# ajpowelsnl/mhm2_proxy

Measured on AMD Instinct MI355X. Metric: k-mers/s (whole node), k=21 150bp reads, higher is better.
Workload: dtype u64

## Files before the change

mhm2_proxy_amd/csrc/kcount_kernels.hip:

```cpp
#include <hip/hip_runtime.h>
#include <type_traits>

#include <algorithm>

#include "kcount_launch.hpp"
#include "kmer_ops.hpp"

namespace mhm {

template <int NL>
constexpr int kTile() {
  return TILE_BASES[NL];
}
template <int NL>
constexpr int kEThreads() {
  return E_THREADS_NL[NL];
}
template <int NL>
constexpr int kPTile() {
  return P_TILE[NL];
}
template <int NL>
constexpr int kPThreads() {
  return P_THREADS[NL];
// ... 1210 lines not shown
#pragma unroll
  for (int j = 0; j < W; j++) {
    const uint32_t i = threadIdx.x + j * NT;
    const uint64_t idx = ch.start + (i < ch.count ? i : ch.count - 1);
    if (RecKind<NL, CMP>::C32) {
      rk[j][0] = (uint64_t)gload((const uint32_t *)src.w[0] + idx);
      rx[j] = (uint32_t)gload(src.ext + idx);
      continue;
    }
    if (RecKind<NL, CMP>::M2) {
      const u32x4 v = gload4((const uint32_t *)src.w[0] + 4 * idx);
      rk[j][0] = (uint64_t)v.x | ((uint64_t)v.y << 32);
      rk[j][NL - 1] = (uint64_t)v.z | ((uint64_t)v.w << 32);
      rx[j] = 0u;
      continue;
    }
#pragma unroll
    for (int w = 0; w < NL; w++) rk[j][w] = gload(src.w[w] + idx);
    rx[j] = PACKED ? 0u : (uint32_t)gload(src.ext + idx);
  }
  if (RecKind<NL, CMP>::C32) {
#pragma unroll
    for (int j = 0; j < W; j++) rk[j][0] |= (uint64_t)rx[j] << 32;
  }
#pragma unroll
  for (int j = 0; j < W; j++) re[j] = PACKED ? (uint32_t)(rk[j][RecKind<NL, CMP>::XW] & 63u) : rx[j];
}

template <int NL, bool PACKED, bool CMP>
__global__ __launch_bounds__(kPThreads<NL>()) void k_part_hist(PartitionParams p) {
  constexpr int NT = kPThreads<NL>(), T = kPTile<NL>(), W = T / NT;
  extern __shared__ __align__(16) uint32_t hist[];
  const uint32_t nf = 1u << p.fine_bits;
  for (uint32_t b = threadIdx.x; b < nf; b += NT) hist[b] = 0;
  uint32_t c;
  if (!xcd_chunk(p, c)) return;
  const SChunk ch = chunk_of<T>(p, c);
  const PlaneSet src = p.srcs[ch.src];
  uint64_t rk[W][NL];
  uint32_t re[W];
  load_chunk<NL, PACKED, CMP, W>(src, ch, rk, re);
  __syncthreads();
#pragma unroll
  for (int j = 0; j < W; j++) {
    if (threadIdx.x + j * NT < ch.count) atomicAdd(&hist[fine_digit<NL, PACKED, CMP>(rk[j], p)], 1u);
  }
  __syncthreads();
  unsigned long long *g = p.fine_hist + (uint64_t)ch.coarse_local * nf;
  for (uint32_t b = threadIdx.x; b < nf; b += NT) {
    const uint32_t c = hist[b];
    if (c) atomicAdd(&g[b], (unsigned long long)c);
  }
}

template <int NL, bool PACKED, bool CMP, int BPT = 8>
__global__ __launch_bounds__(kPThreads<NL>()) void k_part_scatter(PartitionParams p) {
  constexpr int NT = kPThreads<NL>(), T = kPTile<NL>(), W = T / NT;
  static_assert(T % NT == 0 && NT % 64 == 0, "whole records per thread, whole waves");
  extern __shared__ __align__(16) unsigned char smem[];
  const uint32_t nf = 1u << p.fine_bits;
  scatter_clear<NT>((uint32_t *)smem, nf);
  uint32_t c;
  if (!xcd_chunk(p, c)) return;
  const SChunk ch = chunk_of<T>(p, c);
  const PlaneSet src = p.srcs[ch.src];
  if constexpr (RecKind<NL, CMP>::C32) {
    const uint32_t *b32 = (const uint32_t *)src.w[0] + ch.start;
    const uint8_t *b8 = src.ext + ch.start;
    uint32_t lo[W], hi[W];
#pragma unroll
    for (int j = 0; j < W; j++) {
      const uint32_t i = min((uint32_t)(threadIdx.x + j * NT), ch.count - 1u);
      lo[j] = gload(b32 + i);
      hi[j] = gload(b8 + i);
    }
    const uint64_t cmask = (1ull << (EXT_BITS + 2 * p.k - p.coarse_bits - p.fine_bits)) - 1;
#pragma unroll
    for (int j = 0; j < W; j++) {
      uint64_t r[1] = {(uint64_t)lo[j] | ((uint64_t)hi[j] << 32)};
      hi[j] = (threadIdx.x + j * NT < ch.count) ? (1u << 31) | fine_digit<NL, PACKED, CMP>(r, p) : 0u;
      lo[j] = (uint32_t)(r[0] & cmask);
    }
    BinLimit lim{0, 0, 0};
    if (p.coarse_fcap) {
      const uint64_t fc = p.coarse_fcap[ch.coarse_local];
      lim = BinLimit{p.coarse_base[ch.coarse_local], fc, fc};
    }
    __syncthreads();
    scatter_staged_c40<W, NT, false, BPT>(lo, hi, nf, smem, smem + staged_cnt_bytes(nf),
                                     p.fine_cursor + (uint64_t)ch.coarse_local * nf, p.out, lim, p.err);
    return;
  }
  uint64_t rk[W][NL];
  uint32_t re[W], inf[W];
  load_chunk<NL, PACKED, CMP, W>(src, ch, rk, re);
  const uint64_t cmask =
      (1ull << (EXT_BITS + (NL == 1 ? 2 * p.k : RecKind<NL, CMP>::lw(p.k)) - p.coarse_bits - p.fine_bits)) - 1;
#pragma unroll
  for (int j = 0; j < W; j++) {
    inf[j] = (threadIdx.x + j * NT < ch.count)
                 ? ((1u << 31) | (re[j] << 16) | fine_digit<NL, PACKED, CMP>(rk[j], p))
                 : 0u;
    if (CMP) rk[j][0] &= cmask;
  }
  __syncthreads();
  BinLimit lim{0, 0, 0};
  if (p.coarse_fcap) {
    const uint64_t fc = p.coarse_fcap[ch.coarse_local];
    lim = BinLimit{p.coarse_base[ch.coarse_local], fc, fc};
  }
  unsigned long long *cur = p.fine_cursor + (uint64_t)ch.coarse_local * nf;
  constexpr int SF = RecKind<NL, CMP>::M2 ? SF_AOS2 : SF_WORDS;
  scatter_staged<NL, PACKED, W, SF, NT, W * NT, BPT>(rk, inf, nf, smem, smem + staged_cnt_bytes(nf), cur, 1, p.out, lim, p.err);
}

template <int NL, bool PACKED, bool CMP>
__global__ __launch_bounds__(kPThreads<NL>()) void k_sketch(PartitionParams p, unsigned int *hll, unsigned int *fhist) {
  constexpr int NT = kPThreads<NL>(), T = kPTile<NL>(), W = T / NT;
  __shared__ unsigned int reg[SKETCH_M];
  __shared__ unsigned int fh[SKETCH_FH];
  __shared__ unsigned int s_ext;
  if (threadIdx.x == 0) s_ext = 0;
  for (int i = threadIdx.x; i < SKETCH_M; i += NT) reg[i] = 0;
  if (fhist)
    for (int i = threadIdx.x; i < SKETCH_FH; i += NT) fh[i] = 0;
  const SChunk ch = chunk_of<T>(p, blockIdx.x);
  const PlaneSet src = p.srcs[ch.src];
  uint64_t rk[W][NL];
  uint32_t re[W];
  load_chunk<NL, PACKED, CMP, W>(src, ch, rk, re);
  __syncthreads();
  const uint64_t low_mask = CMP ? 63ull : PACKED ? (1ull << (EXT_BITS + p.hbits)) - 1 : 0ull;
  uint32_t ext_adds = 0;
#pragma unroll
  for (int j = 0; j < W; j++) {
    if (threadIdx.x + j * NT >= ch.count) continue;
    ext_adds += (uint32_t)(((re[j] >> 3) & 7u) < 4u) + (uint32_t)((re[j] & 7u) < 4u);
    uint64_t h = 0x9E3779B97F4A7C15ull;
#pragma unroll
    for (int w = 0; w < NL; w++) h = fmix64(h ^ (w == RecKind<NL, CMP>::XW ? rk[j][w] & ~low_mask : rk[j][w]));
    const uint32_t rho = (uint32_t)__clzll(h | (uint64_t)(SKETCH_M - 1)) + 1;
    atomicMax(&reg[h & (SKETCH_M - 1)], rho);
    if (fhist) atomicAdd(&fh[fine_digit<NL, PACKED, CMP>(rk[j], p)], 1u);
  }
  atomicAdd(&s_ext, ext_adds);
  __syncthreads();
  if (fhist)
    for (int i = threadIdx.x; i < SKETCH_FH; i += NT)
      if (fh[i]) atomicAdd(&fhist[i], fh[i]);
  for (int i = threadIdx.x; i < SKETCH_M; i += NT)
    if (reg[i]) {
      atomicMax(&hll[i], reg[i]);
      if (!(blockIdx.x & 1u)) atomicMax(&hll[SKETCH_M + 1 + i], reg[i]);
    }
  if (threadIdx.x == 0 && s_ext) atomicAdd(&hll[SKETCH_M], s_ext);
}

__global__ void k_init_fine(const unsigned long long *coarse_base, const unsigned long long *coarse_fcap, uint32_t n_coarse,
                            int fine_bits, unsigned long long *base, unsigned long long *cursor) {
  const uint64_t i = (uint64_t)blockIdx.x * blockDim.x + threadIdx.x;
  if (i >= ((uint64_t)n_coarse << fine_bits)) return;
  const uint64_t c = i >> fine_bits, d = i & ((1ull << fine_bits) - 1);
  const unsigned long long b = coarse_base[c] + d * coarse_fcap[c];
  base[i] = b;
  cursor[i] = b;
}

__global__ __launch_bounds__(256) void k_count_windows(ReadsView rv, int k, unsigned long long *out, unsigned int *err) {
  __shared__ unsigned long long s_acc[4];
  unsigned long long acc = 0;
  bool bad = false;
  const uint64_t stride = (uint64_t)gridDim.x * blockDim.x;
  for (uint64_t r0 = (uint64_t)blockIdx.x * blockDim.x + threadIdx.x; r0 < rv.n_reads; r0 += 4 * stride) {
    uint64_t a[4], b[4];
#pragma unroll
    for (int u = 0; u < 4; u++) {
      const uint64_t r = r0 + u * stride, rr = r < rv.n_reads ? r : rv.n_reads - 1;
      a[u] = rv.offs[rr];
      b[u] = rv.offs[rr + 1];
    }
#pragma unroll
    for (int u = 0; u < 4; u++) {
      if (r0 + u * stride >= rv.n_reads) break;
      bad |= b[u] < a[u] || b[u] - a[u] > 65535;
      const uint64_t L = b[u] - a[u];
      acc += (b[u] >= a[u] && L > (uint64_t)k + 1) ? L - k - 1 : 0;
    }
  }
  if (blockIdx.x == 0 && threadIdx.x == 0)
    bad |= rv.offs[0] != rv.obase + rv.head || rv.offs[rv.n_reads] - rv.obase != rv.n_bases;
  if (bad) atomicOr(err, 4u);
  acc = wave_sum_u64(acc);
  if ((threadIdx.x & 63) == 0) s_acc[threadIdx.x >> 6] = acc;
  __syncthreads();
  if (threadIdx.x == 0) {
    const unsigned long long t = s_acc[0] + s_acc[1] + s_acc[2] + s_acc[3];
    if (t) atomicAdd(out, t);
  }
}

__global__ __launch_bounds__(256) void k_expand_nibbles(const uint8_t *nib, uint8_t *arena, uint64_t b0, uint64_t n) {
  const uint64_t a0 = b0 & ~15ull, end = b0 + n;
  const uint64_t p0 = a0 + ((uint64_t)blockIdx.x * blockDim.x + threadIdx.x) * 16;
  if (p0 >= end) return;
  uint32_t w[4] = {0, 0, 0, 0};
#pragma unroll
  for (int i = 0; i < 16; i++) {
    const uint64_t p = p0 + i;
    if (p >= b0 && p < end) {
      const uint64_t j = p - b0;
      const uint32_t v = (nib[j >> 1] >> (4 * (uint32_t)(j & 1))) & 15u;
      w[i >> 2] |= ((v & 7u) | ((v >> 3) * 0xf8u)) << (8 * (i & 3));
    }
  }
  if (p0 >= b0 && p0 + 16 <= end) {
    *(uint4 *)(arena + p0) = make_uint4(w[0], w[1], w[2], w[3]);
    return;
  }
#pragma unroll
  for (int i = 0; i < 16; i++) {
    const uint64_t p = p0 + i;
    if (p >= b0 && p < end) arena[p] = (uint8_t)(w[i >> 2] >> (8 * (i & 3)));
  }
}

__global__ __launch_bounds__(256) void k_offs_from_deltas(const uint32_t *d, uint64_t *offs, uint64_t n, uint64_t b0) {
  for (uint64_t i = (uint64_t)blockIdx.x * 256 + threadIdx.x; i < n; i += (uint64_t)gridDim.x * 256) offs[i] = b0 + d[i];
}

__global__ __launch_bounds__(1024) void k_scan(const unsigned long long *in, unsigned long long *base,
                                               unsigned long long *cursor, uint32_t n) {
  __shared__ unsigned long long wsum[17];
  const int tid = threadIdx.x, lane = tid & 63, wid = tid >> 6;
  const uint32_t per = (n + 1023) / 1024;
  const uint32_t lo = min((uint32_t)tid * per, n), hi = min(lo + per, n);
  unsigned long long s = 0;
  for (uint32_t i = lo; i < hi; i++) s += (in[i] + 3) & ~3ull;
  unsigned long long x = s;
#pragma unroll
  for (int d = 1; d < 64; d <<= 1) {
    unsigned long long y = __shfl_up(x, d, 64);
    if (lane >= d) x += y;
  }
  if (lane == 63) wsum[wid] = x;
  __syncthreads();
  if (tid == 0) {
    unsigned long long acc = 0;
    for (int w = 0; w < 16; w++) {
      unsigned long long t = wsum[w];
      wsum[w] = acc;
      acc += t;
    }
  }
  __syncthreads();
  unsigned long long run = wsum[wid] + x - s;
  for (uint32_t i = lo; i < hi; i++) {
    base[i] = run;
    cursor[i] = run;
    run += (in[i] + 3) & ~3ull;
  }
}


template <int NL>
constexpr int count_rpt() {
  return NL == 1 ? 4 : 1;
}

template <int NL>
__device__ __forceinline__ uint32_t slot_hash(const uint64_t *key) {
  if (NL == 1) {
    const uint32_t x = (uint32_t)(key[0] >> 32) * 0x9E3779B1u + (uint32_t)key[0] * 0x85EBCA77u;
    return x ^ (x >> 15);
  }
  uint64_t h = key[0] * 0x9E3779B97F4A7C15ull;
#pragma unroll
  for (int w = 1; w < NL; w++) h = (h ^ (h >> 31) ^ key[w]) * 0xC2B2AE3D27D4EB4Full;
  h ^= h >> 29;
  return (uint32_t)(h >> 32);
}

__device__ __forceinline__ int cmp_group(uint32_t key, int kshl, uint32_t ng) {
  return (int)(__umul24((key << kshl) >> 16, ng) >> 16);
}

template <typename K>
struct CountLds {
  K *keys;
  uint32_t *cnt;
  uint32_t *ext;
  int cap;
  uint32_t *clog;
};

typedef __attribute__((address_space(3))) unsigned int lds_u32_t;
__device__ __forceinline__ uint32_t lds_add_late(unsigned int *p, uint32_t v) {
  lds_u32_t *q = (lds_u32_t *)p;
  asm volatile("" : "+v"(q));
  return __hip_atomic_fetch_add(q, v, __ATOMIC_RELAXED, __HIP_MEMORY_SCOPE_WORKGROUP);
}

#ifndef MHMKC_TAIL_DIV
#define MHMKC_TAIL_DIV 1
#endif
#ifndef MHMKC_TAIL_SLOTS
#define MHMKC_TAIL_SLOTS 4
// ... 1115 lines not shown
  const size_t lds = ((size_t)1 << p.fine_bits) * 4;
  hipError_t e = allow_lds(k_part_hist<NL, PK, CMP>, lds);
  if (e != hipSuccess) return e;
  k_part_hist<NL, PK, CMP><<<dim3(p.grid), dim3(kPThreads<NL>()), lds, s>>>(p);
  return hipGetLastError();
}

template <int NL, bool PK, bool CMP = false>
static hipError_t do_part_scatter(const PartitionParams &p, hipStream_t s) {
  const uint32_t nf = 1u << p.fine_bits;
  const size_t lds = staged_cnt_bytes(nf) + staged_area_bytes(NL, kPTile<NL>(), PK, RecKind<NL, CMP>::C32 ? SF_C32 : SF_WORDS);
  if (nf <= (uint32_t)kPThreads<NL>()) {
    hipError_t e = allow_lds(k_part_scatter<NL, PK, CMP, 1>, lds);
    if (e != hipSuccess) return e;
    k_part_scatter<NL, PK, CMP, 1><<<dim3(p.grid), dim3(kPThreads<NL>()), lds, s>>>(p);
    return hipGetLastError();
  }
  hipError_t e = allow_lds(k_part_scatter<NL, PK, CMP>, lds);
  if (e != hipSuccess) return e;
  k_part_scatter<NL, PK, CMP><<<dim3(p.grid), dim3(kPThreads<NL>()), lds, s>>>(p);
  return hipGetLastError();
}

template <int NL, bool PK, bool CMP = false>
static hipError_t do_count(const CountParams &p, hipStream_t s) {
  const size_t lds = count_lds_bytes(NL, RecKind<NL, CMP>::C32);
  const uint32_t grid = p.grid && p.grid < p.n_buckets ? p.grid : p.n_buckets;
  hipError_t e = p.wide_thr ? allow_lds(k_count<NL, PK, CMP, true>, lds) : allow_lds(k_count<NL, PK, CMP, false>, lds);
  if (e != hipSuccess) return e;
  if (p.wide_thr)
    k_count<NL, PK, CMP, true><<<dim3(grid), dim3(C_THREADS), lds, s>>>(p);
  else
    k_count<NL, PK, CMP, false><<<dim3(grid), dim3(C_THREADS), lds, s>>>(p);
  return hipGetLastError();
}

hipError_t launch_tile_first_read(const ReadsView &r, uint32_t *out, uint32_t n_tiles, int tile, hipStream_t s) {
  if (!n_tiles) return hipSuccess;
  k_tile_first_read<<<dim3((n_tiles + 255) / 256), dim3(256), 0, s>>>(r, out, n_tiles, tile);
  return hipGetLastError();
}

uint64_t read_start_words(uint64_t n_tiles, int nl) {
  const uint64_t T = nl == 1 ? kTile<1>() : nl == 2 ? kTile<2>() : nl == 3 ? kTile<3>() : kTile<4>();
  const uint64_t NG = nl == 1 ? kGroups<1>() : nl == 2 ? kGroups<2>() : nl == 3 ? kGroups<3>() : kGroups<4>();
  return n_tiles * (T / 32) + NG + 2;
}

hipError_t launch_read_start_bits(const ReadsView &r, uint32_t *bits, uint64_t n_words, hipStream_t s) {
  const uint64_t blocks = std::min<uint64_t>(8192, (r.n_reads + 1 + 255) / 256);
  k_read_start_bits<<<dim3((unsigned)blocks), dim3(256), 0, s>>>(r, bits, n_words);
  return hipGetLastError();
}

hipError_t launch_count_windows(const ReadsView &r, int k, unsigned long long *out, unsigned int *err, hipStream_t s) {
  if (!r.n_reads) return hipSuccess;
  const uint64_t blocks = std::min<uint64_t>(2048, (r.n_reads + 1023) / 1024);
  k_count_windows<<<dim3((unsigned)blocks), dim3(256), 0, s>>>(r, k, out, err);
  return hipGetLastError();
}

hipError_t launch_offs_from_deltas(const uint32_t *d, uint64_t *offs, uint64_t n, uint64_t b0, hipStream_t s) {
  if (!n) return hipSuccess;
  k_offs_from_deltas<<<dim3((unsigned)std::min<uint64_t>(4096, (n + 255) / 256)), dim3(256), 0, s>>>(d, offs, n, b0);
  return hipGetLastError();
}

hipError_t launch_expand_nibbles(const uint8_t *nib, uint8_t *arena, uint64_t b0, uint64_t n, hipStream_t s) {
  if (!n) return hipSuccess;
  const uint64_t blocks16 = (b0 + n - (b0 & ~15ull) + 15) / 16;
  k_expand_nibbles<<<dim3((unsigned)((blocks16 + 255) / 256)), dim3(256), 0, s>>>(nib, arena, b0, n);
  return hipGetLastError();
}

__global__ __launch_bounds__(256) void k_inc_fixup(const unsigned long long *coarse_base,
                                                  const unsigned long long *coarse_fcap, int fine_bits,
                                                  unsigned long long *cursor, uint8_t *skip, unsigned int *err) {
  const uint32_t c = blockIdx.x, nf = 1u << fine_bits;
  const unsigned long long b0 = coarse_base[c], fcap = coarse_fcap[c];
  unsigned long long *cur = cursor + ((uint64_t)c << fine_bits);
  int over = 0;
  for (uint32_t f = threadIdx.x; f < nf; f += 256) over |= cur[f] > b0 + (f + 1) * fcap;
  over = __syncthreads_or(over);
  if (over)
    for (uint32_t f = threadIdx.x; f < nf; f += 256) cur[f] = b0 + f * fcap;
  if (threadIdx.x == 0) {
    skip[c] = (uint8_t)over;
    if (c == 0) atomicAnd(err, ~2u);
  }
}

hipError_t launch_inc_fixup(const unsigned long long *coarse_base, const unsigned long long *coarse_fcap,
                            uint32_t n_coarse, int fine_bits, unsigned long long *cursor, uint8_t *skip,
                            unsigned int *err, hipStream_t s) {
  if (!n_coarse) return hipSuccess;
  k_inc_fixup<<<dim3(n_coarse), dim3(256), 0, s>>>(coarse_base, coarse_fcap, fine_bits, cursor, skip, err);
  return hipGetLastError();
}

hipError_t launch_init_fine(const unsigned long long *coarse_base, const unsigned long long *coarse_fcap,
                            uint32_t n_coarse, int fine_bits, unsigned long long *base, unsigned long long *cursor,
                            hipStream_t s) {
  const uint64_t n = (uint64_t)n_coarse << fine_bits;
  if (!n) return hipSuccess;
  k_init_fine<<<dim3((unsigned)((n + 255) / 256)), dim3(256), 0, s>>>(coarse_base, coarse_fcap, n_coarse, fine_bits,
                                                                      base, cursor);
  return hipGetLastError();
}

hipError_t launch_extract_hist(const ExtractParams &p, int nl, bool packed, hipStream_t s) {
  if (!p.n_tiles) return hipSuccess;
  if (p.compact) return MHM_DISPATCH_MIXED(nl, do_extract_hist, (p, s));
  MHM_DISPATCH(nl, packed, do_extract_hist, (p, s));
}

hipError_t launch_extract_scatter(const ExtractParams &p, int nl, bool packed, hipStream_t s) {
  if (!p.n_tiles) return hipSuccess;
  if (p.compact) return MHM_DISPATCH_MIXED(nl, do_extract_scatter, (p, s));
  MHM_DISPATCH(nl, packed, do_extract_scatter, (p, s));
}

hipError_t launch_part_hist(const PartitionParams &p, int nl, bool packed, hipStream_t s) {
  if (!p.n_chunks) return hipSuccess;
  if (p.compact) return MHM_DISPATCH_MIXED(nl, do_part_hist, (p, s));
  MHM_DISPATCH(nl, packed, do_part_hist, (p, s));
}

hipError_t launch_part_scatter(const PartitionParams &p, int nl, bool packed, hipStream_t s) {
  if (!p.n_chunks) return hipSuccess;
  if (p.compact) return MHM_DISPATCH_MIXED(nl, do_part_scatter, (p, s));
  MHM_DISPATCH(nl, packed, do_part_scatter, (p, s));
}

hipError_t launch_chunk_runs(const SRun *runs, uint32_t n_runs, SChunk *chunks, int tile, hipStream_t s) {
  if (!n_runs) return hipSuccess;
  k_chunk_runs<<<dim3(n_runs), dim3(256), 0, s>>>(runs, chunks, tile);
  return hipGetLastError();
}

template <int NL, bool PK, bool CMP = false>
static hipError_t do_sketch(const PartitionParams &p, uint32_t n, unsigned int *hll, bool fh, hipStream_t s) {
  k_sketch<NL, PK, CMP><<<dim3(n), dim3(kPThreads<NL>()), 0, s>>>(p, hll, fh ? hll + SKETCH_WORDS : nullptr);
  return hipGetLastError();
}

hipError_t launch_sketch(const PartitionParams &p, uint32_t n_chunks, unsigned int *hll, int nl, bool packed,
                         hipStream_t s, bool fine_hist) {
  if (!n_chunks) return hipSuccess;
  if (fine_hist && p.fine_bits != SKETCH_FB) return hipErrorInvalidValue;
  if (p.compact) return MHM_DISPATCH_MIXED(nl, do_sketch, (p, n_chunks, hll, fine_hist, s));
  MHM_DISPATCH(nl, packed, do_sketch, (p, n_chunks, hll, fine_hist, s));
}

hipError_t launch_scan(const unsigned long long *in, unsigned long long *base, unsigned long long *cursor, uint32_t n,
                       hipStream_t s) {
  k_scan<<<dim3(1), dim3(1024), 0, s>>>(in, base, cursor, n);
  return hipGetLastError();
}

hipError_t launch_count(const CountParams &p, int nl, bool packed, hipStream_t s) {
  if (!p.n_buckets) return hipSuccess;
  if (p.compact) return MHM_DISPATCH_MIXED(nl, do_count, (p, s));
  MHM_DISPATCH(nl, packed, do_count, (p, s));
}


template <typename V>
__global__ __launch_bounds__(256) void k_seg_gather(const SegCopy *segs, const V *src, V *dst) {
  const SegCopy sc = segs[blockIdx.x];
  const V *s = src + sc.src;
  V *d = dst + sc.dst;
  for (uint64_t i = threadIdx.x; i < sc.n; i += 256) d[i] = s[i];
}

hipError_t launch_seg_gather(const SegCopy *segs, uint32_t n_segs, const void *src, void *dst, int elem_bytes,
                             hipStream_t s) {
  if (!n_segs) return hipSuccess;
  const dim3 grid(n_segs), block(256);
  switch (elem_bytes) {
    case 1: k_seg_gather<uint8_t><<<grid, block, 0, s>>>(segs, (const uint8_t *)src, (uint8_t *)dst); break;
    case 4: k_seg_gather<uint32_t><<<grid, block, 0, s>>>(segs, (const uint32_t *)src, (uint32_t *)dst); break;
    case 8: k_seg_gather<uint2><<<grid, block, 0, s>>>(segs, (const uint2 *)src, (uint2 *)dst); break;
    case 16: k_seg_gather<uint4><<<grid, block, 0, s>>>(segs, (const uint4 *)src, (uint4 *)dst); break;
    default: return hipErrorInvalidValue;
  }
  return hipGetLastError();
}


template <int NL>
static hipError_t do_smer_owner(const SmerParams &p, hipStream_t s) {
  const size_t lds = smer_owner_lds<NL>(p.n_ranks);
  hipError_t e = allow_lds(k_smer_owner<NL>, lds);
  if (e != hipSuccess) return e;
  k_smer_owner<NL><<<dim3(p.n_tiles), dim3(kEThreads<NL>()), lds, s>>>(p);
  return hipGetLastError();
}

template <int NL>
static hipError_t do_smer_pack(const SmerParams &p, hipStream_t s) {
  const size_t lds = smer_pack_lds<NL>(p.n_ranks);
  hipError_t e = allow_lds(k_smer_pack<NL>, lds);
  if (e != hipSuccess) return e;
  k_smer_pack<NL><<<dim3(p.n_tiles), dim3(kEThreads<NL>()), lds, s>>>(p);
  return hipGetLastError();
}

hipError_t launch_smer_owner(const SmerParams &p, int nl, hipStream_t s) {
  if (!p.n_tiles) return hipSuccess;
  if (p.n_ranks < 2 || p.n_ranks > 255 || p.m < 1 || p.m > 28 || p.m > p.k) return hipErrorInvalidValue;
  switch (nl) {
    case 2: return do_smer_owner<2>(p, s);
    case 3: return do_smer_owner<3>(p, s);
    case 4: return do_smer_owner<4>(p, s);
  }
  return hipErrorInvalidValue;
}

hipError_t launch_smer_pack(const SmerParams &p, int nl, hipStream_t s) {
  if (!p.n_tiles) return hipSuccess;
  if (p.n_ranks < 2 || p.n_ranks > 255) return hipErrorInvalidValue;
  switch (nl) {
    case 2: return do_smer_pack<2>(p, s);
    case 3: return do_smer_pack<3>(p, s);
    case 4: return do_smer_pack<4>(p, s);
  }
  return hipErrorInvalidValue;
}

template <int NL, bool PK, bool CMP, bool HIST>
static hipError_t do_smer_extract(const ExtractParams &p, const SmerSource &src, hipStream_t s) {
  constexpr int T = kTile<NL>();
  constexpr int SF = RecKind<NL, CMP>::M2 ? SF_AOS2 : SF_WORDS;
  const size_t lds = HIST ? (size_t)p.n_bins * 4 : staged_cnt_bytes(p.n_bins) + staged_area_bytes(NL, T, PK, SF);
  hipError_t e = allow_lds(k_smer_extract<NL, PK, CMP, HIST>, lds);
  if (e != hipSuccess) return e;
  k_smer_extract<NL, PK, CMP, HIST><<<dim3(p.n_tiles), dim3(kEThreads<NL>()), lds, s>>>(p, src);
  return hipGetLastError();
}

template <bool HIST>
static hipError_t smer_extract_nl(const ExtractParams &p, const SmerSource &src, int nl, bool packed, hipStream_t s) {
  if (p.compact)
    return nl == 2 ? do_smer_extract<2, true, true, HIST>(p, src, s) : nl == 3 ? do_smer_extract<3, true, true, HIST>(p, src, s)
         : nl == 4 ? do_smer_extract<4, true, true, HIST>(p, src, s) : hipErrorInvalidValue;
  switch (nl * 2 + (packed ? 1 : 0)) {
    case 4: return do_smer_extract<2, false, false, HIST>(p, src, s);
    case 5: return do_smer_extract<2, true, false, HIST>(p, src, s);
    case 6: return do_smer_extract<3, false, false, HIST>(p, src, s);
    case 7: return do_smer_extract<3, true, false, HIST>(p, src, s);
    case 8: return do_smer_extract<4, false, false, HIST>(p, src, s);
    case 9: return do_smer_extract<4, true, false, HIST>(p, src, s);
  }
  return hipErrorInvalidValue;
}

hipError_t launch_smer_extract(const ExtractParams &p, const SmerSource &src, int nl, bool packed, bool hist,
                               hipStream_t s) {
  if (!p.n_tiles) return hipSuccess;
  return hist ? smer_extract_nl<true>(p, src, nl, packed, s) : smer_extract_nl<false>(p, src, nl, packed, s);
}

hipError_t launch_smer_rebase(uint64_t *desc, uint64_t n, uint64_t delta, unsigned long long *nwin, hipStream_t s) {
  if (!n) return hipSuccess;
  k_smer_rebase<<<dim3((unsigned)std::min<uint64_t>(4096, (n + 255) / 256)), dim3(256), 0, s>>>(desc, n, delta, nwin);
  return hipGetLastError();
}

hipError_t launch_smer_tiles(const uint64_t *wpre, uint64_t n_smer, uint64_t *tile_first, uint32_t n_tiles, int tile,
                             hipStream_t s) {
  if (!n_smer) return hipSuccess;
  k_smer_tiles<<<dim3((n_tiles + 1 + 255) / 256), dim3(256), 0, s>>>(wpre, n_smer, tile_first, n_tiles, tile);
  return hipGetLastError();
}

}
```

mhm2_proxy_amd/csrc/kcount_launch.hpp:

```cpp
#pragma once
#include <hip/hip_runtime.h>
#include <stdint.h>

namespace mhm {

struct ReadsView {
  const uint8_t *bytes;
  const uint64_t *offs;
  uint64_t n_reads;
  uint64_t n_bases;
  uint64_t obase;
  uint32_t head;
  uint32_t pad;
};

struct PlaneSet {
  uint64_t *w[4];
  uint8_t *ext;
};

struct ExtractParams {
  ReadsView reads;
  const uint32_t *tile_first_read;
  uint32_t n_tiles;
// ... 67 lines not shown
  uint32_t xcd_start[9];
  uint32_t grid;
  const PlaneSet *srcs;
  int k;
  int coarse_bits;
  int fine_bits;
  int hbits;
  int compact;
  unsigned long long *fine_hist;
  unsigned long long *fine_cursor;
  const unsigned long long *coarse_base;
  const unsigned long long *coarse_fcap;
  unsigned int *err;
  PlaneSet out;
};

struct CountParams {
  PlaneSet recs;
  const unsigned long long *bucket_base;
  const unsigned long long *bucket_end;
  int hbits;
  int compact;
  int coarse_bits, fine_bits;
  uint32_t bucket0;
  uint32_t n_buckets;
  uint32_t grid;
  int k;
  int cap;
  int dmin_thres;
  double dyn_mult;
  int wide_thr;
  int nlo;
  uint64_t *out_keys;
  uint16_t *out_counts;
  char *out_left;
  char *out_right;
  unsigned long long *out_cursor;
  unsigned long long out_cap;
  unsigned long long *stats;
  unsigned int *err;
  uint64_t ctg_n;
  const uint64_t *ctg_keys[4];
  const uint32_t *ctg_state;
  const uint32_t *ctg_bucket;
  uint32_t ctg_base;
  PlaneSet spill;
  uint8_t *ctg_done;
  const uint8_t *coarse_skip;
};

__host__ __device__ inline uint32_t ctg_state_word(uint32_t count, uint32_t l, uint32_t r) {
  return (count & 0xffffu) | (l << 16) | (r << 19);
}

struct CtgView {
  const uint8_t *bytes;
  const uint64_t *offs;
  const uint16_t *depth;
  const uint64_t *win_prefix;
  uint64_t n_ctgs;
  uint64_t n_windows;
};

struct CtgOwner {
  int n_ranks, rank, m;
};

size_t ctg_scratch_bytes(uint64_t n_windows, int nl);
hipError_t ctg_prepare(const CtgView &cv, int k, int nl, bool mixed, int qual_cutoff, int dmin_thres,
                       double dyn_mult, int coarse_bits, int fine_bits, uint32_t own_lo, uint32_t own_hi,
                       const CtgOwner &ow, void *scratch, size_t scratch_bytes,
                       uint64_t *const out_keys[4], uint32_t *out_state, uint32_t *out_bucket, uint64_t *n_out,
                       unsigned int *err, hipStream_t s);

enum {
  STAT_DISTINCT = 0,
  STAT_NOUT = 1,
  STAT_PURGED = 2,
  STAT_COUNTSUM = 3,
  STAT_SWEEPS = 4,
  STAT_MAXBUCKET = 5,
  STAT_MISSES = 6,
  STAT_N = 8,
};
constexpr int STAT_ALLOC = 16;
constexpr uint32_t SPILL_RECORDS = 0xC000;
constexpr int DYN_SWEEP_MAX_NL = 2;

constexpr int E_THREADS = 256;
constexpr int E_NSUB = 8;
#ifndef MHMKC_CSPLIT
#define MHMKC_CSPLIT 1
#endif
constexpr int C_SPLIT = MHMKC_CSPLIT;
constexpr int C_THREADS = 1024 / C_SPLIT;
constexpr size_t C_LDS = 163840 / C_SPLIT;

inline int stored_hash_bits(int k, int nl, bool packed) {
  if (!packed) return 0;
  const int room = 64 - 2 * (k - 32 * (nl - 1)) - 6;
  return room >= 16 ? 16 : (room >= 8 ? room : 0);
}

constexpr int TILE_BASES[5] = {0, 4096, 4096, 1536, 2048};
inline int tile_bases(int nl) { return TILE_BASES[nl]; }
constexpr int E_THREADS_NL[5] = {0, 256, 256, 256, 256};
constexpr int P_TILE[5] = {0, 4096, 3072, 4096, 3072};
constexpr int P_THREADS[5] = {0, 256, 512, 512, 512};
inline int chunk_records(int nl) { return P_TILE[nl]; }
constexpr int COUNT_CAP[5] = {0, 5120, 4000, 3264, 2752};
__host__ __device__ constexpr int count_key_bytes(bool cmp) { return cmp ? 4 : 8; }
__host__ __device__ constexpr int count_cap(int nl, bool cmp = false) {
  return ((cmp ? 6144 : COUNT_CAP[nl]) / C_SPLIT) & ~3;
}
__host__ __device__ constexpr size_t count_table_bytes(int nl, bool cmp = false) {
  return (size_t)count_cap(nl, cmp) * (count_key_bytes(cmp) * nl + 4 + 16) + 256;
}
__host__ __device__ constexpr int miss_cap(int nl, bool cmp = false) {
  return (int)(((C_LDS - count_table_bytes(nl, cmp)) / (count_key_bytes(cmp) * nl + 4)) & ~(size_t)63);
}
constexpr int CLAMP_LOG = 64;
__host__ __device__ constexpr size_t count_log_offset(int nl, bool cmp = false) {
  return count_table_bytes(nl, cmp) + (size_t)miss_cap(nl, cmp) * (count_key_bytes(cmp) * nl + 4);
}
__host__ __device__ constexpr size_t count_lds_bytes(int nl, bool cmp = false) {
  return count_log_offset(nl, cmp) + 4 * (size_t)CLAMP_LOG;
}
static_assert(count_lds_bytes(1) <= C_LDS && count_lds_bytes(2) <= C_LDS && count_lds_bytes(3) <= C_LDS &&
                  count_lds_bytes(4) <= C_LDS && count_lds_bytes(1, true) <= C_LDS,
              "k_count LDS budget");

hipError_t launch_tile_first_read(const ReadsView &r, uint32_t *out, uint32_t n_tiles, int tile, hipStream_t s);
hipError_t launch_read_start_bits(const ReadsView &r, uint32_t *bits, uint64_t n_words, hipStream_t s);
uint64_t read_start_words(uint64_t n_tiles, int nl);
hipError_t launch_count_windows(const ReadsView &r, int k, unsigned long long *out, unsigned int *err, hipStream_t s);
hipError_t launch_expand_nibbles(const uint8_t *nib, uint8_t *arena, uint64_t b0, uint64_t n, hipStream_t s);
hipError_t launch_offs_from_deltas(const uint32_t *d, uint64_t *offs, uint64_t n, uint64_t b0, hipStream_t s);
hipError_t launch_inc_fixup(const unsigned long long *coarse_base, const unsigned long long *coarse_fcap,
                            uint32_t n_coarse, int fine_bits, unsigned long long *cursor, uint8_t *skip,
                            unsigned int *err, hipStream_t s);
hipError_t launch_init_fine(const unsigned long long *coarse_base, const unsigned long long *coarse_fcap,
                            uint32_t n_coarse, int fine_bits, unsigned long long *base, unsigned long long *cursor,
                            hipStream_t s);
hipError_t launch_extract_hist(const ExtractParams &p, int nl, bool packed, hipStream_t s);
hipError_t launch_extract_scatter(const ExtractParams &p, int nl, bool packed, hipStream_t s);
hipError_t launch_chunk_runs(const SRun *runs, uint32_t n_runs, SChunk *chunks, int tile, hipStream_t s);
hipError_t launch_part_hist(const PartitionParams &p, int nl, bool packed, hipStream_t s);
hipError_t launch_part_scatter(const PartitionParams &p, int nl, bool packed, hipStream_t s);
constexpr int SKETCH_M = 1024;
constexpr int SKETCH_WORDS = 2 * SKETCH_M + 1;
constexpr int SKETCH_FB = 11, SKETCH_FH = 1 << SKETCH_FB;
hipError_t launch_sketch(const PartitionParams &p, uint32_t n_chunks, unsigned int *hll, int nl, bool packed,
                         hipStream_t s, bool fine_hist = false);
hipError_t launch_scan(const unsigned long long *in, unsigned long long *base, unsigned long long *cursor,
                       uint32_t n, hipStream_t s);
hipError_t launch_count(const CountParams &p, int nl, bool packed, hipStream_t s);
struct SegCopy {
  uint64_t src, dst, n;
};
hipError_t launch_seg_gather(const SegCopy *segs, uint32_t n_segs, const void *src, void *dst, int elem_bytes,
                             hipStream_t s);

constexpr int FQ_CHUNK = 4096;
constexpr uint64_t FQ_MAX_LINE = 2045;
enum { FQ_E_ID = 1, FQ_E_PLUS = 2, FQ_E_NAME = 3, FQ_E_LEN = 4, FQ_E_LONG = 5, FQ_E_CHAR = 6, FQ_E_TRUNC = 7 };
enum { FQ_E_PAIR_NAME = 8, FQ_E_PAIR_NUM = 9, FQ_E_CHAR2 = 10, FQ_E_QUAL = 11, FQ_E_CHAR1 = 12 };
size_t fq_scan_tmp_bytes(uint64_t n_items);
hipError_t fq_scan(void *tmp, size_t tmp_bytes, const unsigned long long *in, unsigned long long *out,
                   uint64_t n_items, hipStream_t s);
hipError_t launch_fq_count(const char *text, uint64_t n, unsigned long long *chunk, hipStream_t s);
hipError_t launch_offs_rebase(unsigned long long *dst, const unsigned long long *src, uint64_t n, unsigned long long delta,
                              hipStream_t s);
constexpr int FQ_LE_BITS = 40;
constexpr uint64_t FQ_LE_MASK = (1ull << FQ_LE_BITS) - 1;
hipError_t launch_fq_lines(const char *text, uint64_t n, const unsigned long long *chunk_base,
                           unsigned long long *line_end, hipStream_t s);
hipError_t launch_fq_pair_records(const char *text, uint64_t n, const unsigned long long *line_end, uint64_t n_rec,
                                  unsigned long long *len, unsigned long long *err, void *desc_buf, hipStream_t s);
hipError_t launch_fq_records(const char *text, uint64_t n, const unsigned long long *line_end, uint64_t n_rec,
                             unsigned long long *len, unsigned long long *err, hipStream_t s);
size_t fq_pair_desc_bytes(uint64_t n_pairs);
hipError_t launch_fq_merge(const char *text, uint64_t n, const unsigned long long *line_end, uint64_t n_pairs,
                           const unsigned long long *rec_offs, int qual_offset, char *scratch, void *desc_buf,
                           uint32_t *pair_info, unsigned long long *out_len, unsigned long long *err,
                           unsigned long long *stats, hipStream_t s);
hipError_t launch_fq_merge_pack(const char *text, const void *desc_buf, uint64_t n_pairs,
                                const unsigned long long *rec_offs, const char *scratch, const uint32_t *pair_info,
                                const unsigned long long *out_offs, int qual_offset, uint8_t *out,
                                unsigned long long *err, hipStream_t s);
hipError_t launch_fq_pack(const char *text, const unsigned long long *line_end, uint64_t n_rec,
                          const unsigned long long *offs, int qual_offset, uint8_t *out, unsigned long long *err,
                          hipStream_t s);

struct OutRows {
  uint64_t *keys;
  uint16_t *counts;
  char *left, *right;
};
inline int minimizer_len_for(int k) { return k * 2 / 3 + 1 < 15 ? 15 : (k * 2 / 3 + 1 > 27 ? 27 : k * 2 / 3 + 1); }
size_t map_order_scratch_bytes(uint64_t n, int nlo);
hipError_t preload_owner_kernels();
size_t map_slots_scratch_bytes(uint64_t n);
hipError_t launch_map_slots(const uint64_t *keys, uint64_t n, int nlo, uint64_t cap, void *scratch, size_t scratch_bytes,
                            uint32_t *slot, uint8_t *tag, hipStream_t s);
hipError_t launch_map_order(const OutRows &in, uint64_t n, int nlo, void *scratch, size_t scratch_bytes, const OutRows &out,
                            hipStream_t s);
hipError_t launch_minimizer_hash(const uint64_t *keys, uint64_t n, int nlo, int k, int m, uint64_t *out, hipStream_t s);
hipError_t launch_owner_hist(const uint64_t *keys, uint64_t n, int nlo, int k, int m, int n_ranks, uint8_t *dest,
                             unsigned long long *hist, hipStream_t s);
hipError_t launch_owner_scatter(const OutRows &in, uint64_t n, int nlo, const uint8_t *dest, int n_ranks,
                                unsigned long long *cursor, const OutRows &out, hipStream_t s);

struct QueryIndex {
  unsigned long long *slots;
  uint64_t mask;
  uint64_t n_rows;
  int shift;
};
hipError_t preload_query_kernels();
inline unsigned query_grid_cap = 0;
inline unsigned query_grid_for(uint64_t n) {
  const uint64_t g = n + 255 < 16384ull * 256 ? (n + 255) / 256 : 16384;
  return (unsigned)(g < 1 ? 1 : (query_grid_cap && query_grid_cap < g ? query_grid_cap : g));
}
inline unsigned merge_grid_cap = 0;
inline uint64_t merge_grid_for(uint64_t blocks) { return merge_grid_cap && merge_grid_cap < blocks ? merge_grid_cap : blocks; }
hipError_t launch_query_build(const uint64_t *keys, uint64_t n, int nl, int nlo, const QueryIndex &ix, hipStream_t s);
hipError_t launch_query_lookup(const uint64_t *q, uint64_t n, bool canonicalize, int k, int nl, int nlo,
                               const QueryIndex &ix, const OutRows &t, uint32_t *rows, uint16_t *counts, char *left,
                               char *right, hipStream_t s);
hipError_t launch_dbjg_links(const OutRows &t, uint64_t n, int k, int nl, int nlo, const QueryIndex &ix, uint32_t *next,
                             uint8_t *status, hipStream_t s);

struct alignas(32) UutigPort {
  uint64_t link, sum, minw0;
  uint32_t dist, minrow;
};
hipError_t launch_uutig_init(const OutRows &t, uint64_t n, int nlo, const uint32_t *next, const uint8_t *status,
                             const uint64_t *list, uint64_t n_items, const UutigPort *cut, uint32_t round, UutigPort *st,
                             hipStream_t s);
hipError_t launch_uutig_jump(const UutigPort *src, UutigPort *dst, uint64_t n, const uint64_t *list, uint64_t n_items,
                             const uint64_t *keys, int nl, int nlo, uint32_t round, unsigned long long *active,
                             hipStream_t s);
hipError_t launch_uutig_active(const UutigPort *st, uint64_t n, uint64_t *list, uint64_t cap, unsigned long long *n_list,
                               hipStream_t s);
hipError_t launch_uutig_starts(const OutRows &t, uint64_t n, int nl, int nlo, const UutigPort *st, uint32_t *row_ctg,
                               uint32_t *row_pos, uint8_t *row_rc, uint32_t *starts, unsigned long long *n_starts,
                               hipStream_t s);
size_t uutig_table_scratch_bytes(uint64_t n_ctgs);
hipError_t launch_uutig_table(const OutRows &t, uint64_t n, int k, int nl, int nlo, const UutigPort *st, uint32_t *starts,
                              uint64_t n_ctgs, void *scratch, size_t scratch_bytes, uint32_t *row_ctg, uint32_t *n_kmers,
                              double *depths, uint64_t *offsets, hipStream_t s);
hipError_t launch_uutig_place(const OutRows &t, uint64_t n, const UutigPort *st, uint32_t *row_ctg, uint32_t *row_pos,
                              uint8_t *row_rc, hipStream_t s);
hipError_t launch_uutig_bases(const OutRows &t, uint64_t n, int k, int nl, int nlo, const uint32_t *row_ctg,
                              const uint32_t *row_pos, const uint8_t *row_rc, const uint64_t *offsets,
                              const uint32_t *n_kmers, uint64_t n_ctgs, uint64_t n_bases, char *seqs, hipStream_t s);

}
```

mhm2_proxy_amd/csrc/mhmkc_host.cpp:

```cpp
#include <hip/hip_runtime.h>
#include <rccl/rccl.h>

#include <algorithm>
#include <atomic>
#include <chrono>
#include <cmath>
#include <cstdarg>
#include <cstdio>
#include <cstdlib>
#include <condition_variable>
#include <cstring>
#include <functional>
#include <map>
#include <string>
#include <vector>
#include <mutex>
#include <thread>

#include <fcntl.h>
#include <immintrin.h>
#include <sched.h>
#include <sys/stat.h>
#include <unistd.h>

#include "../../include/mhmkc.h"
#include "../../include/mhmkc_debug.h"
#include "kcount_launch.hpp"
#include "kmer_ops.hpp"

namespace {

thread_local std::string g_create_error;

std::atomic<uint64_t> g_dev_live{0}, g_dev_peak{0};

struct DebugKnobs {
  int64_t exact = 0;
  int64_t cap = 0;
  int64_t fine_bits = -1;
  int64_t out_cap = -1;
  int64_t fq_read_fail = -1;
  int64_t wide_records = 0;
  int64_t smer = 1;
  int64_t chunk_bytes = 0;
  int64_t d2h_chunk = 0;
  int64_t h2d_threads = 0;
  int64_t h2d_nt = 1;
  int64_t h2d_adapt = 1;
  int64_t local_rounds = 1;
  int64_t h2d_nib = -1;
  int64_t cb0[4] = {0, 0, 0, 0};
  int64_t query_slots_log2 = 0;
};
DebugKnobs g_dbg;

struct DevBuf {
  void *p = nullptr;
  size_t cap = 0;
  hipError_t ensure(size_t bytes) {
    if (bytes <= cap && p) return hipSuccess;
    release();
    size_t want = bytes + bytes / 16 + 4096;
    hipError_t e = hipMalloc(&p, want);
    if (e != hipSuccess) {
      p = nullptr;
      return e;
    }
    cap = want;
    const uint64_t live = g_dev_live.fetch_add(want) + want;
    uint64_t pk = g_dev_peak.load();
    while (live > pk && !g_dev_peak.compare_exchange_weak(pk, live)) {
    }
    return hipSuccess;
  }
  void release() {
    if (p) {
      (void)hipFree(p);
      g_dev_live.fetch_sub(cap);
    }
    p = nullptr;
    cap = 0;
  }
  template <class T>
  T *as() const {
    return (T *)p;
  }
};

struct PinBuf {
  void *p = nullptr;
  size_t cap = 0;
  hipError_t ensure(size_t bytes) {
    if (bytes <= cap && p) return hipSuccess;
    release();
    size_t want = bytes + bytes / 8 + 4096;
    hipError_t e = hipHostMalloc(&p, want, hipHostMallocDefault);
    if (e != hipSuccess) {
      p = nullptr;
      return e;
    }
    cap = want;
    return hipSuccess;
  }
  void release() {
    if (p) (void)hipHostFree(p);
    p = nullptr;
    cap = 0;
  }
  template <class T>
  T *as() const {
    return (T *)p;
  }
};

size_t align_up(size_t x, size_t a) { return (x + a - 1) / a * a; }

constexpr uint32_t NSUB = mhm::E_NSUB;
struct Slab {
  DevBuf buf;
  DevBuf meta;
  PinBuf pin;
  mhm::PlaneSet planes{};
  mhm::ReadsView rv{};
  uint64_t wins = 0;
  uint64_t n = 0;
  uint32_t tiles = 0;
  int qcut = 20;
  bool pending = false;
  hipEvent_t ev = nullptr;
  std::vector<uint64_t> counts;
  std::vector<uint64_t> bases;
  bool recv = false;
  uint32_t bin_lo = 0, bin_hi = 0;
  uint64_t *codes = nullptr, *desc = nullptr;
  uint32_t *good = nullptr;
  std::vector<uint64_t> sw, ss, swb, ssb;
};

struct Arena {
  DevBuf bytes, offs;
};

struct RecvPart {
  DevBuf buf;
  mhm::PlaneSet planes{};
  struct Span {
    uint64_t off;
    std::vector<uint64_t> start;
    std::vector<uint64_t> count;
  };
  std::vector<Span> spans;
};

struct Source {
  mhm::PlaneSet planes{};
  std::vector<uint64_t> start;
  std::vector<uint64_t> count;
};

struct RunTable {
  std::vector<mhm::SRun> runs;
  std::vector<mhm::PlaneSet> ps;
  uint64_t n_chunks = 0, n_c0 = 0, xcd_max = 0, rec_c0 = 0, rec_c0_even = 0;
  uint64_t xcd_start[9] = {0};
};

struct IncRound {
  RunTable rt;
  DevBuf chunks, srcs;
  PinBuf pin;
};

struct Xfer {
  int peer;
  void *ptr;
  uint64_t bytes;
};

struct Prof {
  int stage;
  hipEvent_t a, b;
};

struct D2HStage {
  std::mutex mu;
  PinBuf buf[2];
};
D2HStage &d2h_stage() {
  static D2HStage *s = new D2HStage();
  return *s;
}

constexpr uint64_t CHUNK_BYTES = 128ull << 20;

int host_threads() {
  int n = 16;
  cpu_set_t cs;
  if (sched_getaffinity(0, sizeof cs, &cs) == 0) n = CPU_COUNT(&cs);
  if (const char *e = getenv("OMP_NUM_THREADS")) {
    const int v = atoi(e);
    if (v > 0) n = std::min(n, v);
  }
  return std::max(1, std::min(16, n));
}

class Workers {
 public:
  static Workers &get() {
    static std::mutex mu;
    static Workers *w = nullptr;
    std::lock_guard<std::mutex> g(mu);
    if (!w || w->pid_ != getpid()) w = new Workers(host_threads());
    return *w;
  }
  int size() const { return n_; }
  void run(const std::function<void(int)> &fn) {
    std::lock_guard<std::mutex> job(job_mu_);
    {
      std::lock_guard<std::mutex> g(mu_);
      fn_ = &fn;
      left_ = n_ - 1;
      gen_++;
    }
    cv_.notify_all();
    fn(0);
    std::unique_lock<std::mutex> g(mu_);
    done_cv_.wait(g, [&] { return left_ == 0; });
    fn_ = nullptr;
  }

 private:
  explicit Workers(int n) : n_(n), pid_(getpid()) {
    for (int t = 1; t < n; t++) std::thread([this, t] { loop(t); }).detach();
  }
  void loop(int t) {
    uint64_t seen = 0;
    for (;;) {
      const std::function<void(int)> *fn;
      {
        std::unique_lock<std::mutex> g(mu_);
        cv_.wait(g, [&] { return gen_ != seen; });
        seen = gen_;
        fn = fn_;
      }
      (*fn)(t);
      std::lock_guard<std::mutex> g(mu_);
      if (--left_ == 0) done_cv_.notify_one();
    }
  }
  const int n_;
  const pid_t pid_;
  std::mutex job_mu_, mu_;
  std::condition_variable cv_, done_cv_;
  const std::function<void(int)> *fn_ = nullptr;
  uint64_t gen_ = 0;
  int left_ = 0;
};

void nib_pack_swar(const uint8_t *src, uint64_t n, uint8_t *dst, int qcut, uint64_t i = 0) {
  const uint32_t qc = (uint32_t)std::min(std::max(qcut, 0), 32);
  constexpr uint64_t L = 0x0101010101010101ull;
  const uint64_t bias = (0x80ull - qc) * L;
  for (; i + 8 <= n; i += 8) {
    uint64_t v;
    memcpy(&v, src + i, 8);
    const uint64_t c = v & (7 * L), q = (v >> 3) & (0x1f * L);
    uint64_t x = c | (((q + bias) >> 4) & (8 * L));
    x = (x | (x >> 4)) & 0x00ff00ff00ff00ffull;
    x = (x | (x >> 8)) & 0x0000ffff0000ffffull;
    const uint32_t y = (uint32_t)(x | (x >> 16));
    memcpy(dst + i / 2, &y, 4);
  }
  for (; i < n; i++) {
    const uint32_t b = src[i], v = (b & 7u) | ((b >> 3) >= qc ? 8u : 0u);
    if (i & 1)
      dst[i / 2] |= (uint8_t)(v << 4);
    else
      dst[i / 2] = (uint8_t)v;
  }
}

__attribute__((target("avx2"))) inline __m256i nib_pairs_avx2(__m256i v, __m256i qm1) {
  const __m256i q = _mm256_and_si256(_mm256_srli_epi16(v, 3), _mm256_set1_epi8(0x1f));
  const __m256i ok = _mm256_and_si256(_mm256_cmpgt_epi8(q, qm1), _mm256_set1_epi8(8));
  return _mm256_maddubs_epi16(_mm256_or_si256(_mm256_and_si256(v, _mm256_set1_epi8(7)), ok), _mm256_set1_epi16(0x1001));
}

__attribute__((target("avx2"))) void nib_pack_avx2(const uint8_t *src, uint64_t n, uint8_t *dst, int qcut, bool nt) {
  const __m256i qm1 = _mm256_set1_epi8((char)(std::min(std::max(qcut, 0), 32) - 1));
  uint64_t i = 0;
  if (nt && ((uintptr_t)dst & 31) == 0) {
    for (; i + 64 <= n; i += 64) {
      const __m256i a = nib_pairs_avx2(_mm256_loadu_si256((const __m256i *)(src + i)), qm1);
      const __m256i b = nib_pairs_avx2(_mm256_loadu_si256((const __m256i *)(src + i + 32)), qm1);
      _mm256_stream_si256((__m256i *)(dst + i / 2), _mm256_permute4x64_epi64(_mm256_packus_epi16(a, b), 0xd8));
    }
    _mm_sfence();
  }
  for (; i + 64 <= n; i += 64) {
    const __m256i a = nib_pairs_avx2(_mm256_loadu_si256((const __m256i *)(src + i)), qm1);
    const __m256i b = nib_pairs_avx2(_mm256_loadu_si256((const __m256i *)(src + i + 32)), qm1);
    _mm256_storeu_si256((__m256i *)(dst + i / 2), _mm256_permute4x64_epi64(_mm256_packus_epi16(a, b), 0xd8));
  }
  nib_pack_swar(src, n, dst, qcut, i);
}

void nib_pack(const uint8_t *src, uint64_t n, uint8_t *dst, int qcut, bool nt = true) {
  static const bool avx2 = __builtin_cpu_supports("avx2");
  if (avx2)
    nib_pack_avx2(src, n, dst, qcut, nt);
  else
    nib_pack_swar(src, n, dst, qcut);
}

struct H2DStage {
  std::mutex mu;
  std::vector<PinBuf *> free;
};
H2DStage &h2d_stage() {
  static H2DStage *s = new H2DStage();
  return *s;
}

}

struct mhmkc {
  mhmkc_config cfg{};
  int k = 0, nl = 1, nlo = 1, mlen = 15;
  int dmin = 2;
  bool packed = true;
  bool compact = false;
  bool mixed2 = false;
  bool mixed3 = false;
  bool mixed() const { return compact || mixed2 || mixed3; }
  int cb = 8, fb = 8, hbits = 0;
  uint32_t nb = 256, nf = 256;
  uint32_t own_lo = 0, own_hi = 256;
  int dev = 0;
  int n_cu = 0;
  hipStream_t stream = nullptr, copy_stream = nullptr;
  bool own_stream = false;
  ncclComm_t comm = nullptr;
  mhmkc_transport xp{};
  bool has_xp = false;

  std::vector<Slab *> slabs;
  size_t n_slabs = 0;
  std::vector<Arena *> arenas;
  size_t n_arenas = 0;
  bool xpipe = false;
  int xpieces = 8;
  hipStream_t xstream = nullptr;
  std::vector<RecvPart *> parts;
  size_t n_parts = 0, xq = 0;
  uint64_t x_rounds = 0;
  bool x_all_done = false;
  double x_ms = 0;
  hipEvent_t ev_xdone = nullptr, ev_xext = nullptr;
  std::vector<hipEvent_t> x_ev;
  int xround(Slab *sl, bool done);
  bool inc = false, inc_tried = false;
  hipStream_t pstream = nullptr;
  hipEvent_t ev_pdone = nullptr;
  uint64_t inc_expect = 0, inc_announced = 0;
  uint64_t x_expect_all = 0;
  std::vector<uint64_t> x_r0_coarse;
  uint64_t x_r0_total = 0;
  std::vector<int> x_round_slab;
  std::vector<IncRound *> inc_pool;
  size_t inc_parted = 0;
  double inc_distinct = 0;
  double inc_ext_per_rec = 0;
  mhm::PlaneSet inc_r2{};
  std::vector<uint64_t> inc_cfit;
  hipEvent_t ev_tail0 = nullptr;
  uint64_t inc_out_est = 0;
  int inc_setup();
  int inc_round(size_t r);
  bool lrounds = false;
  size_t lq = 0;
  int local_rounds(bool all);
  hipEvent_t round_event(size_t r) const { return lrounds ? slabs[(size_t)x_round_slab[r]]->ev : x_ev[2 * r + 1]; }
  void round_sources(size_t r, std::vector<Source> &srcs) const;
  int finish_inc(bool &done, uint64_t *n_out_ret);
  void make_runs(const std::vector<Source> &srcs, uint32_t c0, uint32_t c1, int T, RunTable &rt) const;
  int upload_runs(const RunTable &rt, DevBuf &buf, DevBuf &sbuf, hipStream_t s, mhm::PartitionParams &pp,
                  PinBuf *pin = nullptr);
  int fine_layout(const std::vector<uint64_t> &per_coarse, double slack, std::vector<uint64_t> &cfit,
                  uint64_t &r2_size) const;
  int pump();
  int resolve_one(Slab *sl, bool &redo);
  std::vector<hipEvent_t> chunk_ev;
  DevBuf d_nib[3];
  hipEvent_t nib_ev[3] = {nullptr, nullptr, nullptr};
  bool nib_used[3] = {false, false, false};
  hipEvent_t stage_ev[2] = {nullptr, nullptr};
  int add_host_nib(const uint8_t *bytes, const uint64_t *offs, uint64_t n_reads, int qcut, uint64_t chunk);
  DevBuf d_hist, d_tiles, d_tsb, d_err, d_stats, d_fine_hist, d_fine_base, d_fine_cursor, d_chunks, d_srcs;
  DevBuf d_r2, d_out_keys, d_out_counts, d_out_left, d_out_right, d_out_cursor, d_recv, d_xg;
  DevBuf d_hll, d_dest, d_ohist, d_out2_keys, d_out2_counts, d_out2_left, d_out2_right, d_mh;
  DevBuf d_ord;
  mhm::OutRows ord{};
  bool ord_ready = false;
  int order_rows();
  char *ord_scratch = nullptr;
  size_t ord_scratch_bytes = 0;
  DevBuf d_mslot;
  uint64_t map_cap = 0;
  int map_slots(uint64_t cap);
  DevBuf d_qidx, d_links, d_qstage;
  mhm::QueryIndex qidx{};
  bool qidx_ready = false, links_ready = false;
  mhm::OutRows out_rows() const {
    return mhm::OutRows{d_out_keys.as<uint64_t>(), d_out_counts.as<uint16_t>(), d_out_left.as<char>(),
                        d_out_right.as<char>()};
  }
  int query_index();
  int lookup_device(const uint64_t *d_keys, uint64_t n, int canonicalize, uint32_t *d_rows, uint16_t *d_counts,
                    char *d_left, char *d_right);
  int dbjg_links();
  DevBuf d_uctg, d_useq, d_urows, d_ua, d_ub, d_ulist, d_ucnt, d_utbl;
  bool uutigs_ready = false;
  uint64_t u_nctgs = 0, u_nbases = 0;
  mhmkc_uutig_info uinfo{};
  int uutigs();
  int uutigs_build(std::vector<hipEvent_t> &evs);
  void drop_uutig_scratch() {
    d_ua.release();
    d_ub.release();
    d_ulist.release();
    d_ucnt.release();
    d_utbl.release();
  }
  const uint64_t *u_offsets() const { return d_uctg.as<uint64_t>(); }
  const double *u_depths() const { return (const double *)(d_uctg.as<char>() + align_up((u_nctgs + 1) * 8, 256)); }
  const uint32_t *u_nkmers() const { return (const uint32_t *)((const char *)u_depths() + align_up(u_nctgs * 8 + 8, 256)); }
  void drop_query() {
    d_qidx.release();
    d_links.release();
    d_qstage.release();
    d_uctg.release();
    d_useq.release();
    d_urows.release();
    drop_uutig_scratch();
    qidx = mhm::QueryIndex{};
    qidx_ready = links_ready = uutigs_ready = false;
    u_nctgs = u_nbases = 0;
  }
  DevBuf d_spill;
  DevBuf d_cfit;
  DevBuf d_inc_skip;
  double inc_slack = 0;
  bool smer = false;
  DevBuf d_owners, d_rcodes, d_rgood, d_rdesc, d_rnwin, d_rwpre, d_rtiles, d_rtmp;
  mhm::SmerSource rsrc{};
  uint64_t smer_nwin = 0, smer_seen = 0;
  uint32_t smer_tiles = 0;
  Slab *smer_slab = nullptr;
  int smer_build(Slab *sl);
  int smer_exchange(std::vector<Source> &srcs);
  int smer_records(uint32_t lo, uint32_t hi, std::vector<Source> &srcs);
  PinBuf x_send, x_recv;
  DevBuf d_xsend, d_xsegs;
  std::vector<mhm::SegCopy> x_segs;
  uint64_t x_send_cap = 0;
  DevBuf d_fq_text, d_fq_chunk, d_fq_lines, d_fq_len, d_fq_tmp, d_fq_bytes, d_fq_offs, d_fq_err;
  DevBuf d_fqa_bytes, d_fqa_offs;
  DevBuf d_fq_recoffs, d_fq_scratch, d_fq_pairinfo, d_fq_stats, d_fq_desc;
  uint64_t fq_reads = 0, fq_bases = 0;
  int add_fastq(const char *d_text, uint64_t n, bool pairs = false, uint64_t *consumed = nullptr);
  PinBuf fq_file_buf;
  std::vector<uint8_t> ctg_bytes;
  std::vector<uint64_t> ctg_offs{0}, ctg_win{0};
  std::vector<uint16_t> ctg_depth;
  DevBuf d_ctg_bytes, d_ctg_offs, d_ctg_win, d_ctg_depth, d_ctg_scratch, d_ctg_state, d_ctg_bucket, d_ctg_done;
  DevBuf d_ctg_keys[4];
  uint64_t ctg_n = 0;
  int prepare_ctgs();

  std::string err;
  bool finished = false;
  bool began = false;
  bool partial = false;
  uint64_t n_out = 0;
  mhmkc_stats st{};
  bool profiling = false;
  bool prof_heavy_only = false;
  bool prof_open = false;
  std::vector<Prof> prof;
  std::vector<hipEvent_t> ev_pool;
  hipEvent_t ev_begin = nullptr, ev_end = nullptr, ev_h2d0 = nullptr, ev_h2d1 = nullptr;

  int fail(int code, const char *fmt, ...) {
    char buf[512];
    va_list ap;
    va_start(ap, fmt);
    vsnprintf(buf, sizeof buf, fmt, ap);
    va_end(ap);
    err = buf;
    return code;
  }
  int hip_fail(hipError_t e, const char *what) {
    (void)hipGetLastError();
    return fail(MHMKC_EHIP, "%s: %s (%d)", what, hipGetErrorString(e), (int)e);
  }

  hipEvent_t take_event() {
    if (!ev_pool.empty()) {
      hipEvent_t e = ev_pool.back();
      ev_pool.pop_back();
      return e;
    }
    hipEvent_t e = nullptr;
    (void)hipEventCreate(&e);
    return e;
  }
  void prof_begin(int stage, hipStream_t s = nullptr) {
    prof_open = profiling && (!prof_heavy_only || stage == MHMKC_STAGE_ESCAT || stage == MHMKC_STAGE_SSCAT ||
                              stage == MHMKC_STAGE_XCHG || stage == MHMKC_STAGE_COUNT);
    if (!prof_open) return;
    Prof p{stage, take_event(), take_event()};
    (void)hipEventRecord(p.a, s ? s : stream);
    prof.push_back(p);
  }
  void prof_end(hipStream_t s = nullptr) {
    if (!prof_open || prof.empty()) return;
    prof_open = false;
    (void)hipEventRecord(prof.back().b, s ? s : stream);
  }
  void prof_collect() {
    for (auto &p : prof) {
      float ms = 0;
      if (hipEventElapsedTime(&ms, p.a, p.b) == hipSuccess) {
        st.ms_kernel[p.stage] += ms;
        st.launches[p.stage] += 1;
      }
      ev_pool.push_back(p.a);
      ev_pool.push_back(p.b);
    }
    prof.clear();
  }

  int G() const { return cfg.n_ranks; }
  uint32_t owner_lo(int r) const { return (uint32_t)(((uint64_t)r * nb + cfg.n_ranks - 1) / cfg.n_ranks); }
  uint32_t n_owned() const { return own_hi - own_lo; }
  size_t rec_bytes() const { return compact ? 5 : 8 * (size_t)nl + (packed ? 0 : 1); }
  int min_fine_bits() const { return compact ? std::max(0, 2 * k - cb - 26) : 0; }

  int begin_round() {
    if (finished) return fail(MHMKC_ESTATE, "handle already finished; call mhmkc_reset first");
    if (!began) {
      began = true;
      (void)hipEventRecord(ev_begin, stream);
    }
    return MHMKC_OK;
  }

  Slab *new_slab() {
    if (n_slabs == slabs.size()) slabs.push_back(new Slab());
    Slab *sl = slabs[n_slabs++];
    sl->recv = false;
    sl->bin_lo = sl->bin_hi = 0;
    return sl;
  }
  Arena *new_arena() {
    if (n_arenas == arenas.size()) arenas.push_back(new Arena());
    return arenas[n_arenas++];
  }

  hipError_t grow(DevBuf &b, size_t bytes) {
    if (bytes <= b.cap && b.p) return hipSuccess;
    hipError_t e = hipStreamSynchronize(stream);
    return e != hipSuccess ? e : b.ensure(bytes);
  }

  int set_planes(DevBuf &buf, uint64_t n, mhm::PlaneSet &ps, bool fine = false, bool sync = true) {
    const uint64_t m = std::max<uint64_t>(n, 1);
    const size_t plane = align_up(m * (compact ? 4 : 8), 256);
    const size_t extb = (compact ? !fine : !packed) ? align_up(m, 256) : 0;
    const int np = compact ? 1 : nl;
    hipError_t e = sync ? grow(buf, plane * np + extb) : buf.ensure(plane * np + extb);
    if (e != hipSuccess) return hip_fail(e, "allocating record planes");
    char *b = buf.as<char>();
    for (int w = 0; w < 4; w++) ps.w[w] = w < np ? (uint64_t *)(b + plane * w) : nullptr;
    ps.ext = extb ? (uint8_t *)(b + plane * np) : nullptr;
    return MHMKC_OK;
  }

  void shift_planes(mhm::PlaneSet &ps, uint64_t sh) const {
    if (!sh) return;
    if (compact) {
      ps.w[0] = (uint64_t *)((uint32_t *)ps.w[0] - sh);
    } else if (mixed2) {
      ps.w[0] -= 2 * sh;
      if (ps.w[1]) ps.w[1] -= sh;
    } else {
      for (int w = 0; w < 4; w++)
        if (ps.w[w]) ps.w[w] -= sh;
    }
    if (ps.ext) ps.ext -= sh;
  }

  hipError_t d2h(void *dst, const void *src, size_t bytes);

  int add_view(const mhm::ReadsView &rv, uint64_t wins, bool wins_known);
  int extract(Slab *sl, bool exact);
  int resolve_slabs();
  int add_host(const uint8_t *bytes, const uint64_t *offs, uint64_t n_reads, int qcut);
  int allgather_host(const void *send, void *recv, size_t bytes, hipStream_t xs = nullptr);
  int move(const std::vector<Xfer> &snd, const std::vector<Xfer> &rcv, hipStream_t xs = nullptr);
  int exchange(std::vector<Source> &srcs);
  int gather_ctgs(std::vector<uint8_t> &gb, std::vector<uint64_t> &go, std::vector<uint64_t> &gw,
                  std::vector<uint16_t> &gd);
  bool ctg_gathered = false;
  std::vector<uint8_t> ctg_gbytes;
  std::vector<uint64_t> ctg_goffs, ctg_gwin;
  std::vector<uint16_t> ctg_gdepth;
  int handoff();
  int finish(uint64_t *n_out_ret);
  int finish_passes(uint64_t owned) const;
  hipError_t grow_keep(DevBuf &b, size_t used, size_t need);
  int qcut_pending = 20;
};

constexpr double FINE_LOAD = 0.7;
static double hll_estimate(const std::vector<uint32_t> &reg) {
  const double m = (double)reg.size();
  double sum = 0;
  int zeros = 0;
  for (uint32_t r : reg) {
    sum += std::ldexp(1.0, -(int)r);
    zeros += r == 0;
  }
  const double e = 0.7213 / (1.0 + 1.079 / m) * m * m / sum;
  return (e <= 2.5 * m && zeros) ? m * std::log(m / zeros) : e;
}


int mhmkc::extract(Slab *sl, bool exact) {
  const int T = mhm::tile_bases(nl);
  const uint32_t nseg = nb * NSUB;
  hipError_t e;
  if ((e = grow(d_tiles, (size_t)sl->tiles * 4 + 64)) != hipSuccess) return hip_fail(e, "tile index");
  if ((e = grow(d_hist, (size_t)nb * 8 + 64)) != hipSuccess) return hip_fail(e, "histogram");
  if ((e = sl->meta.ensure((size_t)nseg * 8 + 64)) != hipSuccess) return hip_fail(e, "slab cursors");
  if ((e = sl->pin.ensure((size_t)nseg * 8 + 64)) != hipSuccess) return hip_fail(e, "slab cursors (host)");
  sl->counts.assign(nseg, 0);
  sl->bases.assign(nseg + 1, 0);
  mhm::ExtractParams p{};
  p.reads = sl->rv;
  p.tile_first_read = d_tiles.as<uint32_t>();
  p.n_tiles = sl->tiles;
  p.k = k;
  p.qual_cutoff = sl->qcut;
  p.coarse_bits = cb;
  p.n_bins = nb;
  p.hbits = hbits;
  p.compact = mixed();
  p.hist = d_hist.as<unsigned long long>();
  unsigned long long *dcur = sl->meta.as<unsigned long long>();
  p.cursor = dcur;
  p.err = d_err.as<unsigned int>();
  p.ovf = (unsigned int *)(dcur + nseg);
  const bool filt = sl->bin_hi != 0;
  const uint32_t blo = filt ? sl->bin_lo : 0, bhi = filt ? sl->bin_hi : nb;
  p.bin_lo = filt ? blo : 0;
  p.bin_hi = filt ? bhi : 0;
  uint64_t shift = 0;
  if (!sl->recv) {
    prof_begin(MHMKC_STAGE_TILEIDX);
    const uint64_t words = mhm::read_start_words(sl->tiles, nl);
    if ((e = grow(d_tsb, words * 4 + 64)) == hipSuccess) {
      e = mhm::launch_read_start_bits(sl->rv, d_tsb.as<uint32_t>(), words, stream);
      p.tile_starts = d_tsb.as<uint32_t>();
    }
    prof_end();
    if (e != hipSuccess) return hip_fail(e, "tile index");
  }
  if (exact) {
    std::vector<uint64_t> hist(nb);
    prof_begin(MHMKC_STAGE_OTHER);
    e = hipMemsetAsync(d_hist.p, 0, (size_t)nb * 8, stream);
    prof_end();
    if (e != hipSuccess) return hip_fail(e, "memset");
    prof_begin(MHMKC_STAGE_EHIST);
    e = sl->recv ? mhm::launch_smer_extract(p, rsrc, nl, packed, true, stream) : mhm::launch_extract_hist(p, nl, packed, stream);
    prof_end();
    if (e != hipSuccess) return hip_fail(e, "extract_hist");
    if ((e = hipMemcpyAsync(hist.data(), d_hist.p, (size_t)nb * 8, hipMemcpyDeviceToHost, stream)) != hipSuccess ||
        (e = hipStreamSynchronize(stream)) != hipSuccess)
      return hip_fail(e, "extract_hist");
    uint64_t tot = 0;
    for (uint32_t b = 0; b < nb; b++) {
      sl->bases[b * NSUB] = tot;
      tot += hist[b];
      for (uint32_t q = 1; q < NSUB; q++) sl->bases[b * NSUB + q] = tot;
    }
    sl->bases[nseg] = tot;
    p.bin_cap = 0;
  } else {
    const uint64_t expect = sl->wins / nseg;
    const uint64_t cap = align_up(expect + expect / 25 + 1024, 64);
    for (uint32_t i = 0; i <= nseg; i++) sl->bases[i] = (uint64_t)std::min(std::max(i, blo * NSUB), bhi * NSUB) * cap;
    p.bin_cap = cap;
    shift = (uint64_t)blo * NSUB * cap;
  }
  int rc;
  if ((rc = set_planes(sl->buf, sl->bases[nseg] - shift, sl->planes))) return rc;
  shift_planes(sl->planes, shift);
  uint64_t *hc = sl->pin.as<uint64_t>();
  for (uint32_t i = 0; i < nseg; i++) hc[(size_t)(i % NSUB) * nb + i / NSUB] = sl->bases[i];
  hc[nseg] = 0;
  if ((e = hipMemcpyAsync(dcur, hc, (size_t)nseg * 8 + 8, hipMemcpyHostToDevice, stream)) != hipSuccess)
    return hip_fail(e, "cursor H2D");
  p.out = sl->planes;
  prof_begin(MHMKC_STAGE_ESCAT);
  e = sl->recv ? mhm::launch_smer_extract(p, rsrc, nl, packed, false, stream) : mhm::launch_extract_scatter(p, nl, packed, stream);
  prof_end();
  if (e != hipSuccess) return hip_fail(e, "extract_scatter");
  if ((e = hipMemcpyAsync(hc, dcur, (size_t)nseg * 8 + 8, hipMemcpyDeviceToHost, stream)) != hipSuccess)
    return hip_fail(e, "cursor D2H");
  if (!sl->ev && (e = hipEventCreateWithFlags(&sl->ev, hipEventDisableTiming)) != hipSuccess) return hip_fail(e, "slab event");
  if ((e = hipEventRecord(sl->ev, stream)) != hipSuccess) return hip_fail(e, "slab event");
  sl->pending = true;
  return MHMKC_OK;
}

int mhmkc::add_view(const mhm::ReadsView &rv, uint64_t wins, bool wins_known) {
  hipError_t e;
  if (!wins_known) {
    if ((e = grow(d_hist, (size_t)nb * 8 + 64)) != hipSuccess) return hip_fail(e, "histogram");
    unsigned long long *d_wins = d_hist.as<unsigned long long>() + nb;
    unsigned int ef = 0;
    prof_begin(MHMKC_STAGE_TILEIDX);
    e = hipMemsetAsync(d_wins, 0, 8, stream);
    if (e == hipSuccess) e = mhm::launch_count_windows(rv, k, d_wins, d_err.as<unsigned int>(), stream);
    prof_end();
    if (e == hipSuccess) e = hipMemcpyAsync(&wins, d_wins, 8, hipMemcpyDeviceToHost, stream);
    if (e == hipSuccess) e = hipMemcpyAsync(&ef, d_err.p, 4, hipMemcpyDeviceToHost, stream);
    if (e == hipSuccess) e = hipStreamSynchronize(stream);
    if (e != hipSuccess) return hip_fail(e, "window count");
    if (ef & 4u)
      return fail(MHMKC_EINVAL, "device read offsets are not a PackedReads CSR (offs[0] == 0, non-decreasing, reads "
                                "<= 65535 bases, offs[n_reads] == n_bases)");
  }
  if (wins == 0) return MHMKC_OK;
  const int T = mhm::tile_bases(nl);
  const uint64_t tiles64 = (rv.n_bases + T - 1) / T;
  if (tiles64 >= 0x7fffffffull) return fail(MHMKC_EINVAL, "batch too large");
  Slab *sl = new_slab();
  sl->rv = rv;
  sl->wins = wins;
  sl->tiles = (uint32_t)tiles64;
  sl->qcut = qcut_pending;
  sl->n = 0;
  st.occurrences += wins;
  st.slabs++;
  if (inc_announced >= wins) {
    inc_announced -= wins;
  } else {
    inc_expect += wins - inc_announced;
    inc_announced = 0;
  }
  if (smer) return smer_build(sl);
  int rc = extract(sl, g_dbg.exact != 0);
  return rc ? rc : pump();
}

int mhmkc::resolve_one(Slab *sl, bool &redo) {
  const uint32_t nseg = nb * NSUB;
  hipError_t e;
  redo = false;
  if ((e = hipEventSynchronize(sl->ev)) != hipSuccess) return hip_fail(e, "extract");
  const uint64_t *hc = sl->pin.as<uint64_t>();
  if (hc[nseg] & 2u) {
    st.exact_reruns++;
    redo = true;
    return extract(sl, true);
  }
  uint64_t tot = 0;
  for (uint32_t i = 0; i < nseg; i++) {
    sl->counts[i] = hc[(size_t)(i % NSUB) * nb + i / NSUB] - sl->bases[i];
    tot += sl->counts[i];
  }
  if (!sl->bin_hi && tot != sl->wins) return fail(MHMKC_EHIP, "internal: slab holds %llu records, expected %llu",
                                   (unsigned long long)tot, (unsigned long long)sl->wins);
  sl->n = tot;
  sl->pending = false;
  return MHMKC_OK;
}

int mhmkc::resolve_slabs() {
  for (size_t s = 0; s < n_slabs; s++) {
    Slab *sl = slabs[s];
    for (int pass = 0; sl->pending; pass++) {
      bool redo = false;
      int rc = resolve_one(sl, redo);
      if (rc) return rc;
      if (redo && pass) return fail(MHMKC_EHIP, "internal: exact extraction overflowed");
    }
  }
  return MHMKC_OK;
}

int mhmkc::add_host(const uint8_t *bytes, const uint64_t *offs, uint64_t n_reads, int qcut) {
  int rc = begin_round();
  if (rc) return rc;
  if (offs[0] != 0) return fail(MHMKC_EINVAL, "read_offsets[0] must be 0");
  const uint64_t n_bases = offs[n_reads];
  st.reads += n_reads;
  st.bases += n_bases;
  if (n_reads == 0) return MHMKC_OK;
  if (n_reads >= 0xffffffffull) return fail(MHMKC_EINVAL, "at most 2^32-2 reads per batch");
  uint64_t chunk = CHUNK_BYTES;
  if (g_dbg.chunk_bytes) chunk = std::max<uint64_t>(64, (uint64_t)g_dbg.chunk_bytes);
  if (xpipe) {
    uint64_t w = 0;
    for (uint64_t r = 0; r < n_reads; r++) {
      const uint64_t L = offs[r + 1] >= offs[r] ? offs[r + 1] - offs[r] : 0;
      w += L > (uint64_t)k + 1 ? L - k - 1 : 0;
    }
    inc_expect += w;
    inc_announced += w;
  }
  if (g_dbg.h2d_nib > 0 || (g_dbg.h2d_nib < 0 && host_threads() >= 4))
    return add_host_nib(bytes, offs, n_reads, qcut, chunk);
  hipError_t e;
  Arena *ar = new_arena();
  if ((e = grow(ar->bytes, n_bases + 64)) != hipSuccess || (e = grow(ar->offs, (n_reads + 1) * 8)) != hipSuccess)
    return hip_fail(e, "input staging");
  qcut_pending = qcut;
  (void)hipEventRecord(ev_h2d0, stream);
  if ((e = hipStreamWaitEvent(copy_stream, ev_h2d0, 0)) != hipSuccess) return hip_fail(e, "copy stream");
  (void)hipEventRecord(ev_h2d0, copy_stream);
  uint8_t *db = ar->bytes.as<uint8_t>();
  uint64_t *dofs = ar->offs.as<uint64_t>();
  const uint64_t kk = (uint64_t)k;
  size_t n_ev = 0;
  for (uint64_t r0 = 0; r0 < n_reads;) {
    uint64_t r1 = r0, wins = 0;
    const uint64_t b0 = offs[r0];
    while (r1 < n_reads && (r1 == r0 || offs[r1] - b0 < chunk)) {
      const uint64_t a = offs[r1], b = offs[r1 + 1];
      if (b < a) return fail(MHMKC_EINVAL, "read_offsets must be non-decreasing (read %llu)", (unsigned long long)r1);
      if (b - a > 65535)
        return fail(MHMKC_EINVAL, "read %llu longer than 65535 (PackedRead read_len is uint16)", (unsigned long long)r1);
      if (b - a > kk + 1) wins += b - a - kk - 1;
      r1++;
    }
    const uint64_t b1 = offs[r1];
    if (b1 > b0 && (e = hipMemcpyAsync(db + b0, bytes + b0, b1 - b0, hipMemcpyHostToDevice, copy_stream)) != hipSuccess)
      return hip_fail(e, "input H2D");
    if ((e = hipMemcpyAsync(dofs + r0, offs + r0, (r1 - r0 + 1) * 8, hipMemcpyHostToDevice, copy_stream)) != hipSuccess)
      return hip_fail(e, "input H2D");
    if (n_ev == chunk_ev.size()) {
      hipEvent_t ev = nullptr;
      if ((e = hipEventCreateWithFlags(&ev, hipEventDisableTiming)) != hipSuccess) return hip_fail(e, "event");
      chunk_ev.push_back(ev);
    }
    hipEvent_t ev = chunk_ev[n_ev++];
    if ((e = hipEventRecord(ev, copy_stream)) != hipSuccess || (e = hipStreamWaitEvent(stream, ev, 0)) != hipSuccess)
      return hip_fail(e, "chunk event");
    st.h2d_bytes += (b1 - b0) + (r1 - r0 + 1) * 8;
    st.h2d_chunks++;
    mhm::ReadsView rv{};
    rv.obase = b0 & ~15ull;
    rv.head = (uint32_t)(b0 - rv.obase);
    rv.bytes = db + rv.obase;
    rv.offs = dofs + r0;
    rv.n_reads = r1 - r0;
    rv.n_bases = b1 - rv.obase;
    if ((rc = add_view(rv, wins, true))) return rc;
    r0 = r1;
  }
  (void)hipEventRecord(ev_h2d1, copy_stream);
  if ((e = hipStreamSynchronize(copy_stream)) != hipSuccess) return hip_fail(e, "input H2D");
  float ms = 0;
  if (hipEventElapsedTime(&ms, ev_h2d0, ev_h2d1) == hipSuccess) st.ms_h2d = ms;
  return MHMKC_OK;
}

int mhmkc::add_host_nib(const uint8_t *bytes, const uint64_t *offs, uint64_t n_reads, int qcut, uint64_t chunk) {
  const uint64_t n_bases = offs[n_reads];
  Workers &wk = Workers::get();
  const int T = wk.size();
  hipError_t e;
  int rc;
  Arena *ar = new_arena();
  if ((e = grow(ar->bytes, n_bases + 64)) != hipSuccess || (e = grow(ar->offs, (n_reads + 1) * 8)) != hipSuccess)
    return hip_fail(e, "input staging");
  const uint64_t rmax = std::max<uint64_t>(64, chunk / 32);
  const size_t dof = (size_t)align_up(chunk / 2 + 65536 + 64, 64), slot = dof + 4 * (size_t)(rmax + 1);
  for (int s = 0; s < 3; s++) {
    if (slot > d_nib[s].cap) {
      if (nib_used[s] && (e = hipEventSynchronize(nib_ev[s])) != hipSuccess) return hip_fail(e, "nibble slot");
      if ((e = d_nib[s].ensure(slot)) != hipSuccess) return hip_fail(e, "nibble slot");
    }
    if (!nib_ev[s] && (e = hipEventCreateWithFlags(&nib_ev[s], hipEventDisableTiming)) != hipSuccess)
      return hip_fail(e, "event");
  }
  for (int s = 0; s < 2; s++)
    if (!stage_ev[s] && (e = hipEventCreateWithFlags(&stage_ev[s], hipEventDisableTiming)) != hipSuccess)
      return hip_fail(e, "event");
  struct Slots {
    PinBuf *p[2] = {nullptr, nullptr};
    hipStream_t cs;
    ~Slots() {
      (void)hipStreamSynchronize(cs);
      H2DStage &g = h2d_stage();
      std::lock_guard<std::mutex> lk(g.mu);
      for (PinBuf *b : p)
        if (b) g.free.push_back(b);
    }
  } sl;
  sl.cs = copy_stream;
  {
    H2DStage &g = h2d_stage();
    std::lock_guard<std::mutex> lk(g.mu);
    for (PinBuf *&b : sl.p) {
// ... 1018 lines not shown
    for (int pass = 0; sl->pending; pass++) {
      bool redo = false;
      if ((rc = resolve_one(sl, redo))) return rc;
      if (redo && pass) return fail(MHMKC_EHIP, "internal: exact extraction overflowed");
    }
    if (!inc_tried) {
      if (x_rounds == 0) {
        x_r0_coarse.assign(n_owned(), 0);
        x_r0_total = 0;
      }
      for (uint32_t i = 0; i < nb * NSUB; i++) {
        x_r0_coarse[i / NSUB] += sl->counts[i];
        x_r0_total += sl->counts[i];
      }
    }
    x_expect_all = inc_expect;
    x_round_slab.push_back((int)lq);
    x_rounds++;
    lq++;
    if (!inc_tried && x_rounds >= 2 && (double)x_r0_total >= 0.4 * (double)x_expect_all && (rc = inc_setup()))
      return rc;
    if (inc)
      for (; inc_parted < x_rounds && budget > 0; inc_parted++, budget--)
        if ((rc = inc_round(inc_parted))) return rc;
  }
  if (inc)
    for (; inc_parted < x_rounds && budget > 0; inc_parted++, budget--)
      if ((rc = inc_round(inc_parted))) return rc;
  if (all && !inc_tried && x_rounds >= 2) {
    if ((rc = inc_setup())) return rc;
    if (inc)
      for (; inc_parted < x_rounds; inc_parted++)
        if ((rc = inc_round(inc_parted))) return rc;
  }
  return MHMKC_OK;
}

int mhmkc::inc_setup() {
  inc_tried = true;
  const uint32_t no = n_owned();
  if (!pstream || x_expect_all == 0 || x_r0_total == 0 || (n_parts < 1 && !lrounds) || g_dbg.exact || no == 0)
    return MHMKC_OK;
  hipError_t e;
  std::vector<Source> srcs;
  round_sources(0, srcs);
  if (lrounds)
    for (size_t r = 1; r < x_rounds; r++) {
      std::vector<Source> more;
      round_sources(r, more);
      for (auto &src : more) srcs.push_back(std::move(src));
    }
  const int T = mhm::chunk_records(nl);
  IncRound sk;
  make_runs(srcs, 0, 1, T, sk.rt);
  if (!sk.rt.n_c0 || sk.rt.rec_c0 < 4096) return MHMKC_OK;
  mhm::PartitionParams sp{};
  if ((e = hipStreamWaitEvent(pstream, round_event(0), 0)) != hipSuccess) return hip_fail(e, "partition stream");
  int rc = upload_runs(sk.rt, sk.chunks, sk.srcs, pstream, sp);
  if (rc) return rc;
  const bool fh_ok = !(compact && 2 * k - cb < mhm::SKETCH_FB) && !(mixed2 && k - cb < mhm::SKETCH_FB);
  const size_t words = mhm::SKETCH_WORDS + (size_t)mhm::SKETCH_FH;
  std::vector<uint32_t> reg(words);
  if (fh_ok) sp.fine_bits = mhm::SKETCH_FB;
  prof_begin(MHMKC_STAGE_OTHER, pstream);
  if ((e = d_hll.ensure(4 * words + 64)) != hipSuccess || (e = hipMemsetAsync(d_hll.p, 0, 4 * words, pstream)) != hipSuccess ||
      (e = mhm::launch_sketch(sp, (uint32_t)sk.rt.n_c0, d_hll.as<unsigned int>(), nl, packed, pstream, fh_ok)) != hipSuccess)
    return hip_fail(e, "distinct sketch");
  prof_end(pstream);
  if ((e = hipMemcpyAsync(reg.data(), d_hll.p, 4 * words, hipMemcpyDeviceToHost, pstream)) != hipSuccess ||
      (e = hipStreamSynchronize(pstream)) != hipSuccess)
    return hip_fail(e, "sketch D2H");
  sk.chunks.release();
  sk.srcs.release();
  const double d_f = hll_estimate(std::vector<uint32_t>(reg.begin(), reg.begin() + mhm::SKETCH_M));
  const double d_h = hll_estimate(std::vector<uint32_t>(reg.begin() + mhm::SKETCH_M + 1, reg.begin() + mhm::SKETCH_WORDS));
  const double n_f = (double)sk.rt.rec_c0, n_h = (double)sk.rt.rec_c0_even;
  inc_ext_per_rec = (double)reg[mhm::SKETCH_M] / n_f;
  std::vector<uint64_t> per_coarse(no);
  for (uint32_t c = 0; c < no; c++)
    per_coarse[c] = std::max<uint64_t>(x_r0_coarse[c], (uint64_t)((double)x_expect_all * (double)x_r0_coarse[c] / (double)x_r0_total));
  const double n_exp = (double)per_coarse[0];
  const double slope = (n_f > n_h && d_f > d_h) ? (d_f - d_h) / (n_f - n_h) : 0.0;
  const double d_n = std::min(std::max(d_f + slope * (n_exp - n_f), d_f), d_f * n_exp / n_f);
  const uint32_t cap_slots = (uint32_t)mhm::count_cap(nl, compact);
  int f = 4;
  while (f < 11 && d_n / (double)(1u << f) > FINE_LOAD * cap_slots) f++;
  if (g_dbg.fine_bits >= 0) f = (int)std::min<int64_t>(11, g_dbg.fine_bits);
  fb = std::max(f, min_fine_bits());
  nf = 1u << fb;
  double slack = 0.25;
  if (fh_ok) {
    const uint32_t G = 1u << fb, per = 1u << (mhm::SKETCH_FB - fb);
    std::vector<double> ld(G, 0.0);
    for (uint32_t i = 0; i < (uint32_t)mhm::SKETCH_FH; i++) ld[i / per] += reg[mhm::SKETCH_WORDS + i];
    std::sort(ld.begin(), ld.end());
    ld.pop_back();
    double m = 0, v = 0;
    for (double x : ld) m += x;
    m /= (double)ld.size();
    for (double x : ld) v += (x - m) * (x - m);
    v /= (double)ld.size();
    if (m > 0) slack = std::min(2.0, std::max(0.25, 5.0 * std::sqrt(v) / m));
  }
  inc_slack = slack;
  uint64_t r2_size = 0;
  fine_layout(per_coarse, slack, inc_cfit, r2_size);
  size_t fr = 0, tot = 0;
  const double rec_b = compact ? 4.0 : (double)rec_bytes();
  if (hipMemGetInfo(&fr, &tot) != hipSuccess ||
      (double)r2_size * rec_b > 0.7 * (double)fr + (double)d_r2.cap)
    return MHMKC_OK;
  const uint32_t n_fine = no << fb;
  if ((rc = set_planes(d_r2, r2_size, inc_r2, true, false))) return rc;
  if ((e = d_fine_base.ensure((size_t)n_fine * 8)) != hipSuccess ||
      (e = d_fine_cursor.ensure((size_t)n_fine * 8)) != hipSuccess || (e = d_cfit.ensure(16 * (size_t)no + 64)) != hipSuccess)
    return hip_fail(e, "fine layout");
  unsigned long long *cf = d_cfit.as<unsigned long long>();
  if ((e = hipMemcpyAsync(cf, inc_cfit.data(), 16 * (size_t)no, hipMemcpyHostToDevice, pstream)) != hipSuccess ||
      (e = mhm::launch_init_fine(cf, cf + no, no, fb, d_fine_base.as<unsigned long long>(),
                                 d_fine_cursor.as<unsigned long long>(), pstream)) != hipSuccess)
    return hip_fail(e, "fine layout");
  inc_distinct = d_n * no;
  inc = true;
  return MHMKC_OK;
}

int mhmkc::inc_round(size_t r) {
  const uint32_t no = n_owned();
  while (inc_pool.size() <= r) inc_pool.push_back(new IncRound());
  IncRound *ir = inc_pool[r];
  std::vector<Source> srcs;
  round_sources(r, srcs);
  make_runs(srcs, 0, no, mhm::chunk_records(nl), ir->rt);
  if (!ir->rt.n_chunks) return MHMKC_OK;
  hipError_t e;
  if ((e = hipStreamWaitEvent(pstream, round_event(r), 0)) != hipSuccess) return hip_fail(e, "partition stream");
  mhm::PartitionParams pp{};
  int rc = upload_runs(ir->rt, ir->chunks, ir->srcs, pstream, pp, &ir->pin);
  if (rc) return rc;
  unsigned long long *cf = d_cfit.as<unsigned long long>();
  pp.fine_hist = nullptr;
  pp.fine_cursor = d_fine_cursor.as<unsigned long long>();
  pp.coarse_base = cf;
  pp.coarse_fcap = cf + no;
  pp.out = inc_r2;
  prof_begin(MHMKC_STAGE_SSCAT, pstream);
  e = mhm::launch_part_scatter(pp, nl, packed, pstream);
  prof_end(pstream);
  if (e != hipSuccess) return hip_fail(e, "part_scatter");
  st.inc_rounds++;
  return MHMKC_OK;
}

int mhmkc::finish(uint64_t *n_out_ret) {
  if (partial) return fail(MHMKC_ESTATE, "a failed mhmkc_add_fastq_file left part of the file in this round; call mhmkc_reset");
  int rc = begin_round();
  if (rc) return rc;
  ord_ready = false;
  drop_query();
  ctg_gathered = false;
  if ((rc = resolve_slabs())) return rc;
  hipError_t e;
  const uint32_t no = n_owned();
  std::vector<Source> srcs;
  if (smer) {
    if ((rc = smer_exchange(srcs))) return rc;
  } else if (G() > 1 && xpipe) {
    (void)hipEventRecord(ev_xext, stream);
    for (; xq < n_slabs; xq++)
      if ((rc = xround(slabs[xq], xq + 1 == n_slabs))) return rc;
    while (!x_all_done)
      if ((rc = xround(nullptr, true))) return rc;
    (void)hipEventRecord(ev_xdone, xstream);
    if ((e = hipStreamWaitEvent(stream, ev_xdone, 0)) != hipSuccess || (e = hipEventSynchronize(ev_xdone)) != hipSuccess)
      return hip_fail(e, "exchange");
    x_ms = 0;
    for (uint64_t r = 0; r < x_rounds; r++) {
      float ms = 0;
      if (hipEventElapsedTime(&ms, x_ev[2 * r], x_ev[2 * r + 1]) == hipSuccess) x_ms += ms;
    }
    float exposed = 0;
    if (hipEventElapsedTime(&exposed, ev_xext, ev_xdone) != hipSuccess || exposed < 0) exposed = 0;
    st.xchg_rounds = x_rounds;
    st.ms_xchg = x_ms;
    st.ms_xchg_exposed = exposed;
    if (inc) {
      for (; inc_parted < x_rounds; inc_parted++)
        if ((rc = inc_round(inc_parted))) return rc;
      if ((e = hipEventRecord(ev_pdone, pstream)) != hipSuccess || (e = hipStreamWaitEvent(stream, ev_pdone, 0)) != hipSuccess)
        return hip_fail(e, "partition stream");
    }
    if (profiling) {
      st.ms_kernel[MHMKC_STAGE_XCHG] += x_ms;
      st.launches[MHMKC_STAGE_XCHG] += x_rounds;
    }
    for (size_t s = 0; s < n_slabs; s++) {
      Source src;
      src.planes = slabs[s]->planes;
      src.start.assign(slabs[s]->bases.begin() + own_lo * NSUB, slabs[s]->bases.begin() + own_hi * NSUB);
      src.count.assign(slabs[s]->counts.begin() + own_lo * NSUB, slabs[s]->counts.begin() + own_hi * NSUB);
      srcs.push_back(std::move(src));
    }
    for (size_t q = 0; q < n_parts; q++)
      for (auto &sp : parts[q]->spans) {
        Source src;
        src.planes = parts[q]->planes;
        src.start = sp.start;
        src.count = sp.count;
        srcs.push_back(std::move(src));
      }
  } else if (G() > 1) {
    if ((rc = exchange(srcs))) return rc;
  } else {
    if (lrounds && lq > 0) {
      if ((rc = local_rounds(true))) return rc;
      if (inc && ((e = hipEventRecord(ev_pdone, pstream)) != hipSuccess || (e = hipStreamWaitEvent(stream, ev_pdone, 0)) != hipSuccess))
        return hip_fail(e, "partition stream");
    }
    for (size_t s = 0; s < n_slabs; s++) {
      Source src;
      src.planes = slabs[s]->planes;
      src.start.assign(slabs[s]->bases.begin(), slabs[s]->bases.begin() + (size_t)nb * NSUB);
      src.count = slabs[s]->counts;
      srcs.push_back(std::move(src));
    }
  }
  (void)hipEventRecord(ev_tail0, stream);
  uint64_t owned = smer ? smer_nwin : 0;
  for (auto &s : srcs)
    for (uint32_t i = 0; i < no * NSUB; i++) owned += s.count[i];
  st.owned_records = owned;
  st.coarse_record_bytes = rec_bytes();
  st.fine_record_bytes = compact ? 4 : rec_bytes();
  smer_seen = 0;

  const int T = mhm::chunk_records(nl);
  const uint32_t cap_slots = (uint32_t)mhm::count_cap(nl, compact);
  const bool exact_dbg = g_dbg.exact != 0;
  uint64_t out_cap = 0, out_used = 0;
  unsigned long long acc_stats[mhm::STAT_ALLOC] = {0};
  double est_fine = 0;
  unsigned int errf = 0;
  st.fine_buckets = 0;
  int rc_cp = MHMKC_OK;
  static const char *const CLAMP_LOG_FULL =
      "dyn_min_depth < 0.5 with more than 63 saturating extension counters in one hash bucket (DESIGN.md §3.4)";
  auto count_params = [&](uint32_t c0, uint32_t n_fine) {
    mhm::CountParams cp{};
    cp.bucket_base = d_fine_base.as<unsigned long long>();
    cp.bucket_end = d_fine_cursor.as<unsigned long long>();
    cp.hbits = hbits;
    cp.compact = mixed();
    cp.coarse_bits = cb;
    cp.fine_bits = fb;
    cp.bucket0 = (own_lo + c0) << fb;
    cp.n_buckets = n_fine;
    cp.grid = (uint32_t)std::max(0, n_cu * mhm::C_SPLIT);
    cp.k = k;
    cp.cap = mhm::count_cap(nl, compact);
    st.table_slots = (uint64_t)cp.cap;
    if (g_dbg.cap) cp.cap = std::min<int>(cp.cap, (int)std::max<int64_t>(64, g_dbg.cap) & ~3);
    cp.dmin_thres = dmin;
    cp.dyn_mult = 1.0 - cfg.dyn_min_depth;
    cp.wide_thr = (int)(cp.dyn_mult * 65535.0) > 0x8000 || dmin > 0x8000;
    cp.nlo = nlo;
    cp.out_cursor = d_out_cursor.as<unsigned long long>();
    cp.stats = d_stats.as<unsigned long long>();
    cp.err = d_err.as<unsigned int>();
    cp.ctg_n = ctg_n;
    for (int w = 0; w < 4; w++) cp.ctg_keys[w] = w < nl ? d_ctg_keys[w].as<uint64_t>() : nullptr;
    cp.ctg_state = d_ctg_state.as<uint32_t>();
    cp.ctg_bucket = d_ctg_bucket.as<uint32_t>();
    cp.ctg_done = d_ctg_done.as<uint8_t>();
    cp.ctg_base = c0 << fb;
    if (cp.grid && nl <= mhm::DYN_SWEEP_MAX_NL)
      rc_cp = set_planes(d_spill, (uint64_t)cp.grid * mhm::SPILL_RECORDS, cp.spill, true);
    if (rc_cp) cp.grid = 0;
    return cp;
  };
  auto grow_output = [&](uint64_t rows) -> int {
    hipError_t e_;
    if ((e_ = grow(d_out_keys, rows * 8 * nlo)) != hipSuccess || (e_ = grow(d_out_counts, rows * 2)) != hipSuccess ||
        (e_ = grow(d_out_left, rows)) != hipSuccess || (e_ = grow(d_out_right, rows)) != hipSuccess ||
        (e_ = grow(d_out_cursor, 8)) != hipSuccess)
      return hip_fail(e_, "output");
    return MHMKC_OK;
  };

  bool inc_done = false;
  std::vector<std::pair<uint32_t, uint32_t>> ranges;
  if (inc) {
    const uint32_t n_fine = no << fb;
    nf = 1u << fb;
    st.distinct_estimate = (uint64_t)inc_distinct;
    st.inc_slack = inc_slack;
    st.lds_ext_adds = (uint64_t)(inc_ext_per_rec * (double)owned);
    if ((rc = prepare_ctgs())) return rc;
    out_cap = std::min<uint64_t>(owned / 2, (uint64_t)(0.5 * inc_distinct) + (1u << 20));
    if (g_dbg.out_cap >= 0) out_cap = (uint64_t)g_dbg.out_cap;
    out_cap += ctg_n + 1;
    if ((rc = grow_output(out_cap))) return rc;
    mhm::CountParams cp = count_params(0, n_fine);
    if (rc_cp) return rc_cp;
    if ((e = d_inc_skip.ensure((size_t)no + 64)) != hipSuccess) return hip_fail(e, "skip flags");
    unsigned long long *cf = d_cfit.as<unsigned long long>();
    prof_begin(MHMKC_STAGE_OTHER);
    e = mhm::launch_inc_fixup(cf, cf + no, no, fb, d_fine_cursor.as<unsigned long long>(), d_inc_skip.as<uint8_t>(),
                              d_err.as<unsigned int>(), stream);
    prof_end();
    if (e != hipSuccess) return hip_fail(e, "layout fixup");
    cp.recs = inc_r2;
    cp.coarse_skip = d_inc_skip.as<uint8_t>();
    std::vector<uint8_t> skip(no);
    for (int attempt = 0; attempt < 4 && !inc_done; attempt++) {
      cp.out_keys = d_out_keys.as<uint64_t>();
      cp.out_counts = d_out_counts.as<uint16_t>();
      cp.out_left = d_out_left.as<char>();
      cp.out_right = d_out_right.as<char>();
      cp.out_cap = out_cap;
      unsigned long long stats[mhm::STAT_ALLOC], cursor_end = 0;
      const unsigned long long cur0 = 0;
      prof_begin(MHMKC_STAGE_OTHER);
      e = hipMemcpyAsync(d_out_cursor.p, &cur0, 8, hipMemcpyHostToDevice, stream);
      if (e == hipSuccess) e = hipMemsetAsync(d_stats.p, 0, 8 * mhm::STAT_ALLOC, stream);
      if (e == hipSuccess && ctg_n) e = hipMemsetAsync(d_ctg_done.p, 0, ctg_n, stream);
      prof_end();
      if (e != hipSuccess) return hip_fail(e, "count setup");
      prof_begin(MHMKC_STAGE_COUNT);
      e = mhm::launch_count(cp, nl, packed, stream);
      prof_end();
      if (e != hipSuccess) return hip_fail(e, "count");
      (void)hipEventRecord(ev_end, stream);
      if ((e = hipMemcpyAsync(stats, d_stats.p, sizeof stats, hipMemcpyDeviceToHost, stream)) != hipSuccess ||
          (e = hipMemcpyAsync(&errf, d_err.p, 4, hipMemcpyDeviceToHost, stream)) != hipSuccess ||
          (e = hipMemcpyAsync(&cursor_end, d_out_cursor.p, 8, hipMemcpyDeviceToHost, stream)) != hipSuccess ||
          (e = hipMemcpyAsync(skip.data(), d_inc_skip.p, no, hipMemcpyDeviceToHost, stream)) != hipSuccess ||
          (e = hipStreamSynchronize(stream)) != hipSuccess)
        return hip_fail(e, "finish");
      if (errf & 32u) return fail(MHMKC_EUNSUPPORTED, CLAMP_LOG_FULL);
      if (errf & 2u) break;
      if (errf & 16u) {
        out_cap = cursor_end + cursor_end / 16 + 1024;
        if ((rc = grow_output(out_cap))) return rc;
        st.out_reruns++;
        errf &= ~16u;
        if ((e = hipMemcpy(d_err.p, &errf, 4, hipMemcpyHostToDevice)) != hipSuccess) return hip_fail(e, "flag reset");
        continue;
      }
      if (stats[mhm::STAT_N - 1]) return fail(MHMKC_EHIP, "internal: LDS probe bound exceeded");
      for (int i = 0; i < mhm::STAT_ALLOC; i++) acc_stats[i] = stats[i];
      out_used = cursor_end;
      st.fine_buckets = n_fine;
      inc_done = true;
    }
    if (inc_done) {
      for (uint32_t c = 0; c < no; c++) {
        if (!skip[c]) continue;
        st.inc_redone_coarse++;
        if (!ranges.empty() && ranges.back().second == c)
          ranges.back().second = c + 1;
        else
          ranges.push_back({c, c + 1});
      }
    } else {
      st.inc_fallbacks++;
      errf &= ~(2u | 16u);
      if ((e = hipMemcpy(d_err.p, &errf, 4, hipMemcpyHostToDevice)) != hipSuccess) return hip_fail(e, "flag reset");
    }
  }
  if (!inc_done) {
    const int passes = finish_passes(owned);
    for (int q = 0; q < passes; q++)
      ranges.push_back({(uint32_t)((uint64_t)no * q / passes), (uint32_t)((uint64_t)no * (q + 1) / passes)});
  }
  st.finish_passes = (inc_done ? 1 : 0) + (uint64_t)ranges.size();
  for (size_t pass = 0; pass < ranges.size(); pass++) {
    const uint32_t c0 = ranges[pass].first, c1 = ranges[pass].second;
    const uint32_t np_ = c1 - c0;
    if (!np_) continue;
    const size_t n_srcs0 = srcs.size();
    if (smer && (rc = smer_records(own_lo + c0, own_lo + c1, srcs))) return rc;
    std::vector<uint64_t> per_coarse(np_, 0);
    uint64_t owned_p = 0;
    for (auto &s : srcs)
      for (uint32_t i = c0 * NSUB; i < c1 * NSUB; i++) {
        per_coarse[i / NSUB - c0] += s.count[i];
        owned_p += s.count[i];
      }
    for (uint32_t c = 0; c < np_; c++)
      if (per_coarse[c] >= 0xffffffffull)
        return fail(MHMKC_EUNSUPPORTED, "more than 2^32 records in one hash bucket (split the input into batches of ranks)");

    std::vector<mhm::SRun> runs;
    std::vector<mhm::PlaneSet> ps;
    uint64_t n_chunks = 0, n_c0 = 0;
    uint64_t xcd_start[9] = {0};
    for (size_t s = 0; s < srcs.size(); s++) ps.push_back(srcs[s].planes);
    for (uint32_t x = 0; x < 8; x++) {
      xcd_start[x] = n_chunks;
      for (uint32_t c = c0 + ((x + 8 - c0 % 8) % 8); c < c1; c += 8) {
        for (uint32_t q = 0; q < NSUB; q++)
          for (size_t s = 0; s < srcs.size(); s++) {
            const uint32_t i = c * NSUB + q;
            const uint64_t cnt = srcs[s].count[i];
            if (!cnt) continue;
            runs.push_back({srcs[s].start[i], cnt, (uint32_t)s, c - c0, (uint32_t)n_chunks, 0});
            n_chunks += (cnt + T - 1) / T;
          }
        if (c == c0) n_c0 = n_chunks;
      }
    }
    xcd_start[8] = n_chunks;
    if (n_chunks >= 0x7fffffffull) return fail(MHMKC_EINVAL, "too many chunks");
    uint64_t xcd_max = 0;
    for (int x = 0; x < 8; x++) xcd_max = std::max(xcd_max, xcd_start[x + 1] - xcd_start[x]);
    if ((e = grow(d_chunks, align_up(std::max<size_t>(1, runs.size()) * sizeof(mhm::SRun), 256) +
                                sizeof(mhm::SChunk) * (n_chunks + 1) + 256)) !=
        hipSuccess)
      return hip_fail(e, "chunk table");
    mhm::SRun *d_runs = d_chunks.as<mhm::SRun>();
    mhm::SChunk *d_chunk_run = (mhm::SChunk *)(d_chunks.as<char>() + align_up(runs.size() * sizeof(mhm::SRun), 256));
    if ((e = grow(d_srcs, std::max<size_t>(1, ps.size()) * sizeof(mhm::PlaneSet) + 64)) != hipSuccess ||
        (e = grow(d_cfit, 16 * (size_t)np_ + 64)) != hipSuccess)
      return hip_fail(e, "source table");
    unsigned long long *cfit_d = d_cfit.as<unsigned long long>();
    if (!runs.empty()) {
      if ((e = hipMemcpyAsync(d_runs, runs.data(), runs.size() * sizeof(mhm::SRun), hipMemcpyHostToDevice, stream)) !=
          hipSuccess)
        return hip_fail(e, "run table H2D");
      if ((e = mhm::launch_chunk_runs(d_runs, (uint32_t)runs.size(), d_chunk_run, T, stream)) != hipSuccess)
        return hip_fail(e, "chunk index");
    }
    if (!ps.empty() && (e = hipMemcpyAsync(d_srcs.p, ps.data(), ps.size() * sizeof(mhm::PlaneSet),
                                           hipMemcpyHostToDevice, stream)) != hipSuccess)
      return hip_fail(e, "source H2D");

    if (pass == 0 && !inc_done) {
      fb = 4;
      double est = 0;
      if (n_c0) {
        mhm::PartitionParams sp{};
        sp.runs = d_runs;
        sp.chunks = d_chunk_run;
        sp.n_runs = (uint32_t)runs.size();
        sp.n_chunks = (uint32_t)n_chunks;
        sp.srcs = d_srcs.as<mhm::PlaneSet>();
        sp.k = k;
        sp.coarse_bits = cb;
        sp.hbits = hbits;
        sp.compact = mixed();
        std::vector<uint32_t> reg(mhm::SKETCH_M + 1);
        prof_begin(MHMKC_STAGE_OTHER);
        if ((e = grow(d_hll, 4 * mhm::SKETCH_WORDS + 64)) != hipSuccess ||
            (e = hipMemsetAsync(d_hll.p, 0, 4 * mhm::SKETCH_WORDS, stream)) != hipSuccess ||
            (e = mhm::launch_sketch(sp, (uint32_t)n_c0, d_hll.as<unsigned int>(), nl, packed, stream)) != hipSuccess)
          return hip_fail(e, "distinct sketch");
        prof_end();
        if ((e = hipMemcpyAsync(reg.data(), d_hll.p, 4 * mhm::SKETCH_M + 4, hipMemcpyDeviceToHost, stream)) != hipSuccess ||
            (e = hipStreamSynchronize(stream)) != hipSuccess)
          return hip_fail(e, "sketch D2H");
        if (per_coarse[0]) st.lds_ext_adds = (uint64_t)((double)reg[mhm::SKETCH_M] * (double)owned / (double)per_coarse[0]);
        reg.resize(mhm::SKETCH_M);
        est = hll_estimate(reg);
        st.distinct_estimate = (uint64_t)(est * no);
        while (fb < 11 && est / (double)(1u << fb) > FINE_LOAD * cap_slots) fb++;
        est_fine = est;
      } else {
        const uint64_t avg_coarse = owned / std::max<uint32_t>(no, 1);
        while (fb < 11 && (avg_coarse >> fb) > (uint64_t)cap_slots * 4) fb++;
      }
      if (g_dbg.fine_bits >= 0) fb = (int)std::min<int64_t>(11, g_dbg.fine_bits);
      fb = std::max(fb, min_fine_bits());
      nf = 1u << fb;
      est_fine /= nf;
      if ((rc = prepare_ctgs())) return rc;
      out_cap = owned / 2;
      if (est > 0) out_cap = std::min<uint64_t>(out_cap, (uint64_t)(0.5 * est * no) + (1u << 20));
      if (g_dbg.out_cap >= 0) out_cap = (uint64_t)g_dbg.out_cap;
      out_cap += ctg_n + 1;
      if ((rc = grow_output(out_cap))) return rc;
    }
    const uint32_t n_fine = np_ * nf;
    st.fine_buckets += n_fine;

    std::vector<uint64_t> cfit(2 * (size_t)np_);
    uint64_t r2_size = 0;
    for (uint32_t c = 0; c < np_; c++) {
      const uint64_t ex = per_coarse[c] >> fb;
      const uint64_t fcap = align_up(ex + ex / 4 + 256, 16);
      cfit[c] = r2_size;
      cfit[np_ + c] = fcap;
      r2_size += fcap << fb;
    }
    if ((e = hipMemcpyAsync(cfit_d, cfit.data(), 16 * (size_t)np_, hipMemcpyHostToDevice, stream)) != hipSuccess)
      return hip_fail(e, "layout H2D");
    if ((e = grow(d_fine_hist, (size_t)n_fine * 8)) != hipSuccess) return hip_fail(e, "fine histogram");
    if ((e = grow(d_fine_base, (size_t)n_fine * 8)) != hipSuccess) return hip_fail(e, "fine bases");
    if ((e = grow(d_fine_cursor, (size_t)n_fine * 8)) != hipSuccess) return hip_fail(e, "fine cursor");

    mhm::PartitionParams pp{};
    pp.runs = d_runs;
    pp.chunks = d_chunk_run;
    pp.n_runs = (uint32_t)runs.size();
    pp.n_chunks = (uint32_t)n_chunks;
    for (int x = 0; x < 9; x++) pp.xcd_start[x] = (uint32_t)xcd_start[x];
    pp.grid = (uint32_t)(8 * xcd_max);
    pp.srcs = d_srcs.as<mhm::PlaneSet>();
    pp.k = k;
    pp.coarse_bits = cb;
    pp.fine_bits = fb;
    pp.hbits = hbits;
    pp.compact = mixed();
    pp.fine_hist = d_fine_hist.as<unsigned long long>();
    pp.fine_cursor = d_fine_cursor.as<unsigned long long>();
    pp.err = d_err.as<unsigned int>();

    mhm::CountParams cp = count_params(c0, n_fine);
    if (rc_cp) return rc_cp;
    bool exact = exact_dbg || inc_done;
    unsigned long long stats[mhm::STAT_ALLOC], cursor_end = 0;
    for (int attempt = 0;; attempt++) {
      if (attempt >= 4) return fail(MHMKC_EHIP, "internal: finish pass %d did not settle", pass);
      mhm::PlaneSet r2{};
      if (exact) {
        if ((rc = set_planes(d_r2, owned_p + 3 * (uint64_t)n_fine + 4, r2, true))) return rc;
      } else {
        if ((rc = set_planes(d_r2, r2_size, r2, true))) return rc;
      }
      cp.out_keys = d_out_keys.as<uint64_t>();
      cp.out_counts = d_out_counts.as<uint16_t>();
      cp.out_left = d_out_left.as<char>();
      cp.out_right = d_out_right.as<char>();
      cp.out_cap = out_cap;
      const unsigned long long cur0 = out_used;
      prof_begin(MHMKC_STAGE_OTHER);
      e = hipMemcpyAsync(d_out_cursor.p, &cur0, 8, hipMemcpyHostToDevice, stream);
      if (e == hipSuccess) e = hipMemsetAsync(d_stats.p, 0, 8 * mhm::STAT_ALLOC, stream);
      if (e == hipSuccess && ctg_n) e = hipMemsetAsync(d_ctg_done.p, 0, ctg_n, stream);
      if (e == hipSuccess && exact) e = hipMemsetAsync(d_fine_hist.p, 0, (size_t)n_fine * 8, stream);
      if (e == hipSuccess && !exact)
        e = mhm::launch_init_fine(cfit_d, cfit_d + np_, np_, fb, d_fine_base.as<unsigned long long>(),
                                  d_fine_cursor.as<unsigned long long>(), stream);
      prof_end();
      if (e != hipSuccess) return hip_fail(e, "fine layout");
      if (exact) {
        pp.coarse_base = nullptr;
        pp.coarse_fcap = nullptr;
        prof_begin(MHMKC_STAGE_SHIST);
        e = mhm::launch_part_hist(pp, nl, packed, stream);
        prof_end();
        if (e != hipSuccess) return hip_fail(e, "part_hist");
        prof_begin(MHMKC_STAGE_OTHER);
        e = mhm::launch_scan(d_fine_hist.as<unsigned long long>(), d_fine_base.as<unsigned long long>(),
                             d_fine_cursor.as<unsigned long long>(), n_fine, stream);
        prof_end();
        if (e != hipSuccess) return hip_fail(e, "scan");
      } else {
        pp.coarse_base = cfit_d;
        pp.coarse_fcap = cfit_d + np_;
      }
      pp.out = r2;
      prof_begin(MHMKC_STAGE_SSCAT);
      e = mhm::launch_part_scatter(pp, nl, packed, stream);
      prof_end();
      if (e != hipSuccess) return hip_fail(e, "part_scatter");
      cp.recs = r2;
      prof_begin(MHMKC_STAGE_COUNT);
      e = mhm::launch_count(cp, nl, packed, stream);
      prof_end();
      if (e != hipSuccess) return hip_fail(e, "count");
      (void)hipEventRecord(ev_end, stream);
      if ((e = hipMemcpyAsync(stats, d_stats.p, sizeof stats, hipMemcpyDeviceToHost, stream)) != hipSuccess ||
          (e = hipMemcpyAsync(&errf, d_err.p, 4, hipMemcpyDeviceToHost, stream)) != hipSuccess ||
          (e = hipMemcpyAsync(&cursor_end, d_out_cursor.p, 8, hipMemcpyDeviceToHost, stream)) != hipSuccess ||
          (e = hipStreamSynchronize(stream)) != hipSuccess)
        return hip_fail(e, "finish");
      if (errf & 32u) return fail(MHMKC_EUNSUPPORTED, CLAMP_LOG_FULL);
      if (!(errf & (2u | 16u))) break;
      if (errf & 2u) {
        exact = true;
        st.exact_reruns++;
      } else if (errf & 16u) {
        const uint64_t need = cursor_end + cursor_end / 16 + 1024;
        if ((e = grow_keep(d_out_keys, out_used * 8 * nlo, need * 8 * nlo)) != hipSuccess ||
            (e = grow_keep(d_out_counts, out_used * 2, need * 2)) != hipSuccess ||
            (e = grow_keep(d_out_left, out_used, need)) != hipSuccess ||
            (e = grow_keep(d_out_right, out_used, need)) != hipSuccess)
          return hip_fail(e, "output growth");
        out_cap = need;
        st.out_reruns++;
      }
      errf &= ~(2u | 16u);
      if ((e = hipMemcpy(d_err.p, &errf, 4, hipMemcpyHostToDevice)) != hipSuccess) return hip_fail(e, "flag reset");
    }
    if (stats[mhm::STAT_N - 1]) return fail(MHMKC_EHIP, "internal: LDS probe bound exceeded");
    for (int i = 0; i < mhm::STAT_ALLOC; i++)
      acc_stats[i] = i == mhm::STAT_MAXBUCKET ? std::max(acc_stats[i], stats[i]) : acc_stats[i] + stats[i];
    out_used = cursor_end;
    srcs.resize(n_srcs0);
  }
  if (smer && smer_seen != smer_nwin)
    return fail(MHMKC_EHIP, "internal: the finish passes extracted %llu of %llu received windows",
                (unsigned long long)smer_seen, (unsigned long long)smer_nwin);
  float ms = 0;
  if (hipEventElapsedTime(&ms, ev_begin, ev_end) == hipSuccess) st.ms_total = ms;
  if (hipEventElapsedTime(&ms, ev_tail0, ev_end) == hipSuccess) st.ms_finish_tail = ms;
  finished = true;
  if (errf & 1u) return fail(MHMKC_EBADCHAR, "input byte with a base code > 4 (not A,C,G,T,N)");
  if (errf & 8u) return fail(MHMKC_EHIP, "internal: supermer spans inconsistent");
#if MHMKC_STAMP
  {
    const char *names[6] = {"clear", "loadwait", "insert", "barrier", "overflow", "finalize"};
    double tot = 0;
    for (int i = 0; i < 6; i++) tot += (double)acc_stats[8 + i];
    fprintf(stderr, "k_count stamps:");
    for (int i = 0; i < 6; i++) fprintf(stderr, " %s %.1f%%", names[i], tot > 0 ? 100.0 * acc_stats[8 + i] / tot : 0.0);
    fprintf(stderr, " (total %.3g wave-cycles); workgroup cycles mean %.4g max %.4g\n", tot,
            (double)acc_stats[14] / std::max(1, n_cu), (double)acc_stats[15]);
  }
#endif
  st.distinct = acc_stats[mhm::STAT_DISTINCT];
  st.n_out = acc_stats[mhm::STAT_NOUT];
  st.purged = acc_stats[mhm::STAT_PURGED];
  st.count_sum = acc_stats[mhm::STAT_COUNTSUM];
  st.overflow_sweeps = acc_stats[mhm::STAT_SWEEPS];
  st.max_bucket = acc_stats[mhm::STAT_MAXBUCKET];
  st.lds_misses = acc_stats[mhm::STAT_MISSES];
  st.dropped = 0;
  n_out = st.n_out;
  if (n_out != out_used) return fail(MHMKC_EHIP, "internal: output rows %llu, cursor %llu", (unsigned long long)n_out,
                                     (unsigned long long)out_used);
  if (cfg.output_owner == MHMKC_OWNER_MINIMIZER && G() > 1 && !smer) {
    if ((rc = handoff())) return rc;
  }
  st.device_bytes = g_dev_live.load();
  st.device_bytes_peak = g_dev_peak.load();
  prof_collect();
  if (n_out_ret) *n_out_ret = n_out;
  return MHMKC_OK;
}

hipError_t mhmkc::d2h(void *dst, const void *src, size_t bytes) {
  const size_t CH = g_dbg.d2h_chunk > 0 ? (size_t)g_dbg.d2h_chunk : 8ull << 20;
  hipError_t e;
  hipPointerAttribute_t pa{};
  const bool pinned = hipPointerGetAttributes(&pa, dst) == hipSuccess && pa.type == hipMemoryTypeHost;
  (void)hipGetLastError();
  if (bytes < 2 * CH || pinned) {
    if ((e = hipMemcpyAsync(dst, src, bytes, hipMemcpyDeviceToHost, stream)) != hipSuccess) return e;
    return hipStreamSynchronize(stream);
  }
  D2HStage &stg = d2h_stage();
  std::lock_guard<std::mutex> lock(stg.mu);
  if ((e = stg.buf[0].ensure(CH)) != hipSuccess || (e = stg.buf[1].ensure(CH)) != hipSuccess) return e;
  hipEvent_t ev[2] = {take_event(), take_event()};
  const size_t n_ch = (bytes + CH - 1) / CH;
  auto drain = [&](size_t c) {
    const size_t off = c * CH, len = std::min(CH, bytes - off);
    const char *sp = stg.buf[c & 1].as<char>();
    char *dp = (char *)dst + off;
    auto cut = [&](int t) { return t >= 4 ? len : std::min(len, (len / 4 * (size_t)t) & ~(size_t)63); };
    std::thread th[3];
    for (int t = 1; t < 4; t++) {
      const size_t a = cut(t), b = cut(t + 1);
      th[t - 1] = std::thread([=] { if (b > a) memcpy(dp + a, sp + a, b - a); });
    }
    memcpy(dp, sp, cut(1));
    for (auto &x : th) x.join();
  };
  e = hipSuccess;
  for (size_t c = 0; c < n_ch && e == hipSuccess; c++) {
    const size_t off = c * CH, len = std::min(CH, bytes - off);
    if (c >= 2 && (e = hipEventSynchronize(ev[c & 1])) != hipSuccess) break;
    if ((e = hipMemcpyAsync(stg.buf[c & 1].p, (const char *)src + off, len, hipMemcpyDeviceToHost, stream)) != hipSuccess ||
        (e = hipEventRecord(ev[c & 1], stream)) != hipSuccess)
      break;
    if (c >= 1) {
      if ((e = hipEventSynchronize(ev[(c - 1) & 1])) != hipSuccess) break;
      drain(c - 1);
    }
  }
  if (e == hipSuccess && (e = hipEventSynchronize(ev[(n_ch - 1) & 1])) == hipSuccess) drain(n_ch - 1);
  ev_pool.push_back(ev[0]);
  ev_pool.push_back(ev[1]);
  return e;
}

namespace {
struct HostPool {
  std::mutex mu;
  std::map<void *, size_t> live;
  std::multimap<size_t, void *> free_;
  size_t free_bytes = 0;
};
HostPool &host_pool() {
  static HostPool *p = new HostPool();
  return *p;
}
constexpr size_t HOST_POOL_KEEP = 2ull << 30;
}


extern "C" {

int mhmkc_abi_version(void) { return MHMKC_ABI_VERSION; }

#ifndef MHMKC_BUILD_ID
#define MHMKC_BUILD_ID "unknown"
#endif
__attribute__((used)) static const char k_build_marker[] = "MHMKC_BUILD_ID=" MHMKC_BUILD_ID;
const char *mhmkc_build_id(void) { return k_build_marker + 15; }

int mhmkc_config_init(mhmkc_config *cfg) {
  if (!cfg) return MHMKC_EINVAL;
  memset(cfg, 0, sizeof *cfg);
  cfg->k = 21;
  cfg->n_longs = 0;
  cfg->qual_offset = 33;
  cfg->qual_cutoff = 20;
  cfg->dmin_thres = 2;
  cfg->dyn_min_depth = 0.9;
  cfg->device = -1;
  cfg->rank = 0;
  cfg->n_ranks = 1;
  cfg->comm_id = nullptr;
  cfg->stream = nullptr;
  cfg->output_owner = MHMKC_OWNER_HASH;
  cfg->minimizer_len = 0;
  return MHMKC_OK;
}

int mhmkc_comm_id(uint8_t out[MHMKC_COMM_ID_BYTES]) {
  if (!out) return MHMKC_EINVAL;
  ncclUniqueId id;
  ncclResult_t r = ncclGetUniqueId(&id);
  if (r != ncclSuccess) {
    g_create_error = std::string("ncclGetUniqueId: ") + ncclGetErrorString(r);
    return MHMKC_ERCCL;
  }
  static_assert(sizeof(ncclUniqueId) == MHMKC_COMM_ID_BYTES, "unique id size");
  memcpy(out, &id, MHMKC_COMM_ID_BYTES);
  return MHMKC_OK;
}

int mhmkc_create(mhmkc_t *out, const mhmkc_config *cfg) {
  if (!out || !cfg) {
    g_create_error = "null argument";
    return MHMKC_EINVAL;
  }
  *out = nullptr;
  const int k = cfg->k;
  if (k < 1 || k > 127) {
    g_create_error = "k must be in [1, 127]";
    return MHMKC_EINVAL;
  }
  if (k % 32 == 0) {
    g_create_error = "k % 32 == 0 is not supported (EMPTY-slot aliasing, see DESIGN.md)";
    return MHMKC_EUNSUPPORTED;
  }
  const int nl = k / 32 + 1;
  const int nlo = cfg->n_longs ? cfg->n_longs : nl;
  if (nlo < nl || nlo > 8) {
    g_create_error = "n_longs must be 0 or in [k/32+1, 8]";
    return MHMKC_EINVAL;
  }
  if (cfg->qual_cutoff < 0 || cfg->qual_cutoff > 32 || (cfg->qual_offset != 33 && cfg->qual_offset != 64)) {
    g_create_error = "qual_offset must be 33 or 64 and qual_cutoff in [0, 32]";
    return MHMKC_EINVAL;
  }
  if (cfg->dmin_thres < 0 || cfg->dmin_thres > 32768) {
    g_create_error = "dmin_thres must be in [0, 32768] (DESIGN.md §3.4)";
    return MHMKC_EUNSUPPORTED;
  }
  if (!(cfg->dyn_min_depth >= 0.0 && cfg->dyn_min_depth <= 1.0)) {
    g_create_error = "dyn_min_depth must be in [0, 1]";
    return MHMKC_EINVAL;
  }
  if (cfg->n_ranks < 1 || cfg->n_ranks > 255 || cfg->rank < 0 || cfg->rank >= cfg->n_ranks) {
    g_create_error = "bad rank / n_ranks (1..255 ranks)";
    return MHMKC_EINVAL;
  }
  if (cfg->output_owner != MHMKC_OWNER_HASH && cfg->output_owner != MHMKC_OWNER_MINIMIZER) {
    g_create_error = "output_owner must be MHMKC_OWNER_HASH or MHMKC_OWNER_MINIMIZER";
    return MHMKC_EINVAL;
  }
  const int mlen = cfg->minimizer_len ? cfg->minimizer_len : mhm::minimizer_len_for(k);
  if (cfg->output_owner == MHMKC_OWNER_MINIMIZER && (mlen < 1 || mlen > 28 || mlen > k)) {
    g_create_error = "minimizer_len must be in [1, min(k, 28)] (Kmer::get_minimizer_fast)";
    return MHMKC_EINVAL;
  }
  mhmkc *h = new mhmkc();
  h->cfg = *cfg;
  h->k = k;
  h->nl = nl;
  h->nlo = nlo;
  h->mlen = mlen;
  h->dmin = cfg->dmin_thres;
  h->qcut_pending = cfg->qual_cutoff;
  h->packed = mhm::ext_packs(k, nl);
  h->hbits = mhm::stored_hash_bits(k, nl, h->packed);
  h->smer = cfg->output_owner == MHMKC_OWNER_MINIMIZER && cfg->n_ranks > 1 && nl >= 2 && g_dbg.smer != 0;
  int extra = 0;
  while ((1 << extra) < cfg->n_ranks && extra < 3) extra++;
  if (h->smer) extra = 0;
  const int cb_knob = (int)g_dbg.cb0[nl >= 3 ? 3 : nl];
  const int cb0 = cb_knob ? cb_knob : nl >= 3 ? 7 : 8;
  const int cb_min = nl >= 3 ? 7 : nl == 2 ? std::max(1, k - 58) : 1;
  if (cb0 < cb_min || cb0 + extra > 11) {
    delete h;
    g_create_error = "coarse bits out of range: " + std::to_string(cb0) + " + " + std::to_string(extra) +
                     " rank bits for k = " + std::to_string(k) + " (at least " + std::to_string(cb_min) +
                     ", at most 11 with the rank bits)";
    return MHMKC_EUNSUPPORTED;
  }
  h->cb = cb0 + extra;
  const bool wide = g_dbg.wide_records != 0;
  h->compact = mhm::compact_ok(k, nl) && 2 * k - h->cb <= 34 && !wide;
  if (h->compact) h->hbits = 0;
  h->mixed2 = mhm::mixed2_ok(k, nl) && !wide;
  if (h->mixed2) {
    h->packed = true;
    h->hbits = 0;
  }
  h->mixed3 = mhm::mixed3_ok(k, nl) && !wide;
  if (h->mixed3) {
    h->packed = true;
    h->hbits = 0;
  }
  h->nb = 1u << h->cb;
  h->own_lo = h->smer ? 0 : h->owner_lo(cfg->rank);
  h->own_hi = h->smer ? h->nb : h->owner_lo(cfg->rank + 1);
  hipError_t e;
  if (cfg->device >= 0) {
    if ((e = hipSetDevice(cfg->device)) != hipSuccess) {
      g_create_error = std::string("hipSetDevice: ") + hipGetErrorString(e);
      delete h;
      return MHMKC_EHIP;
    }
  }
  (void)hipGetDevice(&h->dev);
  if (hipDeviceGetAttribute(&h->n_cu, hipDeviceAttributeMultiprocessorCount, h->dev) != hipSuccess) h->n_cu = 0;
  if (cfg->stream) {
    h->stream = (hipStream_t)cfg->stream;
  } else {
    if ((e = hipStreamCreateWithFlags(&h->stream, hipStreamNonBlocking)) != hipSuccess) {
      g_create_error = std::string("hipStreamCreate: ") + hipGetErrorString(e);
      delete h;
      return MHMKC_EHIP;
    }
    h->own_stream = true;
  }
  if ((e = hipStreamCreateWithFlags(&h->copy_stream, hipStreamNonBlocking)) != hipSuccess ||
      (e = hipEventCreate(&h->ev_begin)) != hipSuccess || (e = hipEventCreate(&h->ev_end)) != hipSuccess ||
      (e = hipEventCreate(&h->ev_h2d0)) != hipSuccess || (e = hipEventCreate(&h->ev_h2d1)) != hipSuccess ||
      (e = h->d_err.ensure(16)) != hipSuccess || (e = h->d_stats.ensure(8 * mhm::STAT_ALLOC)) != hipSuccess ||
      (e = hipMemset(h->d_err.p, 0, 16)) != hipSuccess) {
    g_create_error = std::string("init: ") + hipGetErrorString(e);
    mhmkc_destroy(h);
    return MHMKC_EHIP;
  }
  const char *xp_env = getenv("MHMKC_XPIPE");
  h->xpipe = cfg->n_ranks > 1 && !h->smer && xp_env && atoi(xp_env);
  h->lrounds = cfg->n_ranks == 1 && !h->smer && g_dbg.local_rounds != 0;
  if (const char *env = getenv("MHMKC_XPIECES")) h->xpieces = std::max(1, std::min(64, atoi(env)));
  if ((e = hipEventCreate(&h->ev_tail0)) != hipSuccess ||
      (h->xpipe && ((e = hipStreamCreateWithFlags(&h->xstream, hipStreamNonBlocking)) != hipSuccess ||
                    (e = hipEventCreate(&h->ev_xdone)) != hipSuccess || (e = hipEventCreate(&h->ev_xext)) != hipSuccess)) ||
      ((h->xpipe || h->lrounds) && ((e = hipStreamCreateWithFlags(&h->pstream, hipStreamNonBlocking)) != hipSuccess ||
                                    (e = hipEventCreateWithFlags(&h->ev_pdone, hipEventDisableTiming)) != hipSuccess))) {
    g_create_error = std::string("exchange stream: ") + hipGetErrorString(e);
    mhmkc_destroy(h);
    return MHMKC_EHIP;
  }
  (void)mhm::preload_owner_kernels();
  (void)mhm::preload_query_kernels();
  if (cfg->n_ranks > 1 && cfg->comm_id) {
    ncclUniqueId id;
    memcpy(&id, cfg->comm_id, sizeof id);
    ncclResult_t r = ncclCommInitRank(&h->comm, cfg->n_ranks, id, cfg->rank);
    if (r != ncclSuccess) {
      g_create_error = std::string("ncclCommInitRank: ") + ncclGetErrorString(r);
      h->comm = nullptr;
      mhmkc_destroy(h);
      return MHMKC_ERCCL;
    }
  }
  *out = h;
  return MHMKC_OK;
}

void mhmkc_destroy(mhmkc_t h) {
  if (!h) return;
  if (h->stream) (void)hipStreamSynchronize(h->stream);
  if (h->copy_stream) (void)hipStreamSynchronize(h->copy_stream);
  if (h->xstream) (void)hipStreamSynchronize(h->xstream);
  if (h->pstream) (void)hipStreamSynchronize(h->pstream);
  if (h->comm) ncclCommDestroy(h->comm);
  for (IncRound *q : h->inc_pool) {
    q->chunks.release();
    q->srcs.release();
    q->pin.release();
    delete q;
  }
  if (h->pstream) (void)hipStreamDestroy(h->pstream);
  if (h->ev_pdone) (void)hipEventDestroy(h->ev_pdone);
  if (h->ev_tail0) (void)hipEventDestroy(h->ev_tail0);
  for (RecvPart *q : h->parts) {
    q->buf.release();
    delete q;
  }
  for (hipEvent_t ev : h->x_ev) (void)hipEventDestroy(ev);
  if (h->ev_xdone) (void)hipEventDestroy(h->ev_xdone);
  if (h->ev_xext) (void)hipEventDestroy(h->ev_xext);
  if (h->xstream) (void)hipStreamDestroy(h->xstream);
  if (h->smer_slab) h->slabs.push_back(h->smer_slab);
  for (Slab *s : h->slabs) {
    if (s->ev) (void)hipEventDestroy(s->ev);
    s->buf.release();
    s->meta.release();
    s->pin.release();
    delete s;
  }
  for (Arena *a : h->arenas) {
    a->bytes.release();
    a->offs.release();
    delete a;
  }
  DevBuf *bufs[] = {&h->d_hist,     &h->d_tiles,      &h->d_err,        &h->d_stats,      &h->d_fine_hist,
                    &h->d_fine_base, &h->d_fine_cursor, &h->d_chunks,    &h->d_srcs,       &h->d_r2,
                    &h->d_out_keys, &h->d_out_counts, &h->d_out_left,   &h->d_out_right,  &h->d_out_cursor,
                    &h->d_recv,     &h->d_xg,         &h->d_hll,        &h->d_dest,       &h->d_ohist,
                    &h->d_out2_keys, &h->d_out2_counts, &h->d_out2_left, &h->d_out2_right, &h->d_mh, &h->d_ord,
                    &h->d_spill,      &h->d_cfit,       &h->d_xsend,      &h->d_xsegs,
                    &h->d_owners, &h->d_rcodes, &h->d_rgood, &h->d_rdesc, &h->d_rnwin, &h->d_rwpre, &h->d_rtiles,
                    &h->d_rtmp,
                    &h->d_fqa_bytes, &h->d_fqa_offs,
                    &h->d_fq_text,  &h->d_fq_chunk,   &h->d_fq_lines,   &h->d_fq_len,     &h->d_fq_tmp,
                    &h->d_fq_bytes, &h->d_fq_offs,    &h->d_fq_err};
  for (DevBuf *b : bufs) b->release();
  h->drop_query();
  DevBuf *cbufs[] = {&h->d_ctg_bytes, &h->d_ctg_offs, &h->d_ctg_win,   &h->d_ctg_depth, &h->d_ctg_scratch,
                     &h->d_ctg_state, &h->d_ctg_bucket, &h->d_ctg_done, &h->d_ctg_keys[0], &h->d_ctg_keys[1],
                     &h->d_ctg_keys[2], &h->d_ctg_keys[3]};
  for (DevBuf *b : cbufs) b->release();
  h->x_send.release();
  h->x_recv.release();
  h->fq_file_buf.release();
  for (auto &p : h->prof) {
    h->ev_pool.push_back(p.a);
    h->ev_pool.push_back(p.b);
  }
  for (hipEvent_t ev : h->ev_pool) (void)hipEventDestroy(ev);
  for (hipEvent_t ev : h->chunk_ev) (void)hipEventDestroy(ev);
  for (DevBuf &b : h->d_nib) b.release();
  hipEvent_t evs[] = {h->ev_begin,  h->ev_end,    h->ev_h2d0,    h->ev_h2d1,       h->nib_ev[0],
                      h->nib_ev[1], h->nib_ev[2], h->stage_ev[0], h->stage_ev[1]};
  for (hipEvent_t ev : evs)
    if (ev) (void)hipEventDestroy(ev);
  if (h->copy_stream) (void)hipStreamDestroy(h->copy_stream);
  if (h->own_stream && h->stream) (void)hipStreamDestroy(h->stream);
  delete h;
}

int mhmkc_add_reads_device(mhmkc_t h, const uint8_t *d_bytes, const uint64_t *d_offs, uint64_t n_reads,
                           uint64_t n_bases) {
  if (!h) return MHMKC_EINVAL;
  if (n_reads && (!d_bytes || !d_offs)) return h->fail(MHMKC_EINVAL, "null device buffer");
  int rc = h->begin_round();
  if (rc) return rc;
  h->st.reads += n_reads;
  h->st.bases += n_bases;
  if (n_reads == 0) return MHMKC_OK;
  if (n_reads >= 0xffffffffull) return h->fail(MHMKC_EINVAL, "at most 2^32-2 reads per batch");
  h->qcut_pending = h->cfg.qual_cutoff;
  const uint64_t P = (uint64_t)h->xpieces;
  if (h->xpipe && P > 1 && n_reads >= 64 * P) {
    std::vector<uint64_t> cut(P + 1);
    hipError_t e = hipSuccess;
    for (uint64_t i = 0; i <= P && e == hipSuccess; i++)
      e = hipMemcpyAsync(&cut[i], d_offs + n_reads * i / P, 8, hipMemcpyDeviceToHost, h->stream);
    if (e == hipSuccess) e = hipStreamSynchronize(h->stream);
    if (e != hipSuccess) return h->hip_fail(e, "read offsets");
    if (cut[0] != 0)
      return h->fail(MHMKC_EINVAL, "device read offsets are not a PackedReads CSR (offs[0] == 0, non-decreasing, reads "
                                   "<= 65535 bases, offs[n_reads] == n_bases)");
    std::vector<mhm::ReadsView> rvs(P);
    for (uint64_t i = 0; i < P; i++) {
      const uint64_t r0 = n_reads * i / P, r1 = n_reads * (i + 1) / P;
      if (cut[i + 1] < cut[i] || cut[P] != n_bases)
        return h->fail(MHMKC_EINVAL, "device read offsets are not a PackedReads CSR (offs[n_reads] == n_bases)");
      mhm::ReadsView &rv = rvs[i];
      rv = mhm::ReadsView{};
      rv.obase = cut[i] & ~15ull;
      rv.head = (uint32_t)(cut[i] - rv.obase);
      rv.bytes = d_bytes + rv.obase;
      rv.offs = d_offs + r0;
      rv.n_reads = r1 - r0;
      rv.n_bases = cut[i + 1] - rv.obase;
    }
    std::vector<uint64_t> wins(P, 0);
    unsigned int ef = 0;
    if ((e = h->grow(h->d_hist, (size_t)(h->nb + P) * 8 + 64)) != hipSuccess) return h->hip_fail(e, "histogram");
    unsigned long long *d_wins = h->d_hist.as<unsigned long long>() + h->nb;
    h->prof_begin(MHMKC_STAGE_TILEIDX);
    e = hipMemsetAsync(d_wins, 0, 8 * P, h->stream);
    for (uint64_t i = 0; i < P && e == hipSuccess; i++)
      e = mhm::launch_count_windows(rvs[i], h->k, d_wins + i, h->d_err.as<unsigned int>(), h->stream);
    h->prof_end();
    if (e == hipSuccess) e = hipMemcpyAsync(wins.data(), d_wins, 8 * P, hipMemcpyDeviceToHost, h->stream);
    if (e == hipSuccess) e = hipMemcpyAsync(&ef, h->d_err.p, 4, hipMemcpyDeviceToHost, h->stream);
    if (e == hipSuccess) e = hipStreamSynchronize(h->stream);
    if (e != hipSuccess) return h->hip_fail(e, "window count");
    if (ef & 4u)
      return h->fail(MHMKC_EINVAL, "device read offsets are not a PackedReads CSR (offs[0] == 0, non-decreasing, reads "
                                   "<= 65535 bases, offs[n_reads] == n_bases)");
    uint64_t tot = 0;
    for (uint64_t w : wins) tot += w;
    h->inc_expect += tot;
    h->inc_announced += tot;
    for (uint64_t i = 0; i < P; i++)
      if ((rc = h->add_view(rvs[i], wins[i], true))) return rc;
    return MHMKC_OK;
  }
  mhm::ReadsView rv{d_bytes, d_offs, n_reads, n_bases, 0, 0, 0};
  return h->add_view(rv, 0, false);
}

int mhmkc_wait_stream(mhmkc_t h, void *stream) {
  if (!h) return MHMKC_EINVAL;
  hipEvent_t ev = h->take_event();
  hipError_t e = hipEventRecord(ev, (hipStream_t)stream);
  if (e == hipSuccess) e = hipStreamWaitEvent(h->stream, ev, 0);
  h->ev_pool.push_back(ev);
  return e == hipSuccess ? MHMKC_OK : h->hip_fail(e, "wait_stream");
}

int mhmkc::add_fastq(const char *d_text, uint64_t n, bool pairs, uint64_t *consumed) {
  int rc = begin_round();
  if (rc) return rc;
  if (consumed) *consumed = 0;
  fq_reads = fq_bases = 0;
  if (pairs) st.fq_pairs = st.fq_merged = st.fq_ambiguous = st.fq_overlap_bases = 0;
  if (n == 0) return MHMKC_OK;
  if (n > mhm::FQ_LE_MASK) return fail(MHMKC_EINVAL, "FASTQ text larger than 2^40 bytes in one call");
  if ((rc = resolve_slabs())) return rc;
  hipError_t e;
  const uint64_t nch = (n + mhm::FQ_CHUNK - 1) / mhm::FQ_CHUNK;
  if ((e = grow(d_fq_chunk, (nch + 1) * 16)) != hipSuccess) return hip_fail(e, "fastq chunk counts");
  unsigned long long *cnt = d_fq_chunk.as<unsigned long long>(), *cbase = cnt + nch + 1;
  size_t tmp_bytes = mhm::fq_scan_tmp_bytes(nch + 1);
  if ((e = grow(d_fq_tmp, tmp_bytes)) != hipSuccess) return hip_fail(e, "fastq scan scratch");
  prof_begin(MHMKC_STAGE_OTHER);
  e = hipMemsetAsync(cnt + nch, 0, 8, stream);
  if (e == hipSuccess) e = mhm::launch_fq_count(d_text, n, cnt, stream);
  if (e == hipSuccess) e = mhm::fq_scan(d_fq_tmp.p, tmp_bytes, cnt, cbase, nch + 1, stream);
  prof_end();
  if (e != hipSuccess) return hip_fail(e, "fastq newline count");
  unsigned long long newlines = 0;
  char last = 0;
  if ((e = hipMemcpyAsync(&newlines, cbase + nch, 8, hipMemcpyDeviceToHost, stream)) != hipSuccess ||
      (e = hipMemcpyAsync(&last, d_text + n - 1, 1, hipMemcpyDeviceToHost, stream)) != hipSuccess ||
      (e = hipStreamSynchronize(stream)) != hipSuccess)
    return hip_fail(e, "fastq newline count D2H");
  const uint64_t all_lines = newlines + (last != '\n' ? 1 : 0);
  const uint64_t lines = consumed ? (pairs ? newlines / 8 * 8 : newlines / 4 * 4) : all_lines;
  const uint64_t R = lines / 4;
  if (consumed && R == 0) return MHMKC_OK;
  if ((e = grow(d_fq_lines, std::max<uint64_t>(all_lines, 1) * 8)) != hipSuccess) return hip_fail(e, "fastq lines");
  if ((e = grow(d_fq_len, (R + 1) * 8)) != hipSuccess || (e = grow(d_fq_offs, (R + 1) * 8)) != hipSuccess ||
      (e = grow(d_fq_err, 8)) != hipSuccess)
    return hip_fail(e, "fastq records");
  const size_t tmp2 = mhm::fq_scan_tmp_bytes(R + 1);
  if (tmp2 > tmp_bytes) {
    if ((e = grow(d_fq_tmp, tmp2)) != hipSuccess) return hip_fail(e, "fastq scan scratch");
    tmp_bytes = tmp2;
  }
  unsigned long long *lend = d_fq_lines.as<unsigned long long>(), *len = d_fq_len.as<unsigned long long>();
  unsigned long long *offs = d_fq_offs.as<unsigned long long>(), *err_d = d_fq_err.as<unsigned long long>();
  const unsigned long long n_end = n;
  prof_begin(MHMKC_STAGE_OTHER);
  e = mhm::launch_fq_lines(d_text, n, cbase, lend, stream);
  if (e == hipSuccess && !consumed && last != '\n')
    e = hipMemcpyAsync(lend + lines - 1, &n_end, 8, hipMemcpyHostToDevice, stream);
  if (e == hipSuccess) e = hipMemsetAsync(err_d, 0xff, 8, stream);
  if (e == hipSuccess && pairs) {
    if ((e = grow(d_fq_desc, mhm::fq_pair_desc_bytes(R / 2))) == hipSuccess)
      e = mhm::launch_fq_pair_records(d_text, n, lend, R, len, err_d, d_fq_desc.p, stream);
  } else if (e == hipSuccess) {
    e = mhm::launch_fq_records(d_text, n, lend, R, len, err_d, stream);
  }
  if (e == hipSuccess) e = mhm::fq_scan(d_fq_tmp.p, tmp_bytes, len, offs, R + 1, stream);
  prof_end();
  if (e != hipSuccess) return hip_fail(e, "fastq records");
  unsigned long long n_bases = 0;
  if ((e = hipMemcpyAsync(&n_bases, offs + R, 8, hipMemcpyDeviceToHost, stream)) != hipSuccess ||
      (e = hipStreamSynchronize(stream)) != hipSuccess)
    return hip_fail(e, "fastq records D2H");
  uint64_t R_out = R;
  if (!pairs) {
    if ((e = grow(d_fq_bytes, std::max<uint64_t>(n_bases, 1) + 64)) != hipSuccess) return hip_fail(e, "fastq bytes");
// ... 837 lines not shown
  uinfo.n_ctgs = n_ctgs;
  uinfo.n_bases = n_bases;
  uinfo.ms_links = had_links ? 0 : ms(t_l, t_l1);
  uinfo.ms_succ = ms(t0, t1);
  uinfo.ms_rank = ms(t1, t2);
  uinfo.ms_cycles = ms(t2, t3);
  uinfo.ms_table = ms(t3, t4);
  uinfo.ms_rows = ms(t4, t5);
  uinfo.ms_total = ms(t0, t5);
  uinfo.scratch_bytes = d_ua.cap + d_ub.cap + d_ucnt.cap + d_ulist.cap + d_utbl.cap;
  uinfo.kept_bytes = d_uctg.cap + d_useq.cap + d_urows.cap;
  return MHMKC_OK;
}

int mhmkc::uutigs() {
  if (uutigs_ready) return MHMKC_OK;
  if (n_out >= 0xffffffffull) return fail(MHMKC_EUNSUPPORTED, "table queries: at most 2^32-2 rows");
  uinfo = mhmkc_uutig_info{};
  std::vector<hipEvent_t> evs;
  const int rc = uutigs_build(evs);
  if (rc) (void)hipStreamSynchronize(stream);
  for (hipEvent_t ev : evs) (void)hipEventDestroy(ev);
  drop_uutig_scratch();
  if (rc) {
    d_uctg.release();
    d_useq.release();
    d_urows.release();
    u_nctgs = u_nbases = 0;
  } else {
    uutigs_ready = true;
  }
  st.device_bytes = g_dev_live.load();
  st.device_bytes_peak = g_dev_peak.load();
  return rc;
}

static int uutigs_need(mhmkc_t h) {
  if (!h) return MHMKC_EINVAL;
  if (h->cfg.n_ranks > 1) return h->fail(MHMKC_EUNSUPPORTED, "uutigs: single-rank handles only");
  if (!h->finished) return h->fail(MHMKC_ESTATE, "uutigs before finish");
  return h->uutigs();
}

int mhmkc_uutigs(mhmkc_t h, uint64_t *n_ctgs, uint64_t *n_bases) {
  int rc = uutigs_need(h);
  if (rc) return rc;
  if (n_ctgs) *n_ctgs = h->u_nctgs;
  if (n_bases) *n_bases = h->u_nbases;
  return MHMKC_OK;
}

int mhmkc_uutigs_device(mhmkc_t h, const uint64_t **d_offsets, const char **d_seqs, const double **d_depths,
                        uint64_t *n_ctgs, uint64_t *n_bases) {
  int rc = uutigs_need(h);
  if (rc) return rc;
  if (d_offsets) *d_offsets = h->u_offsets();
  if (d_seqs) *d_seqs = h->u_nbases ? h->d_useq.as<char>() : nullptr;
  if (d_depths) *d_depths = h->u_nctgs ? h->u_depths() : nullptr;
  if (n_ctgs) *n_ctgs = h->u_nctgs;
  if (n_bases) *n_bases = h->u_nbases;
  return MHMKC_OK;
}

int mhmkc_uutigs_fetch(mhmkc_t h, uint64_t *offsets, char *seqs, double *depths, uint32_t *n_kmers) {
  int rc = uutigs_need(h);
  if (rc) return rc;
  const uint64_t nc = h->u_nctgs, nb = h->u_nbases;
  hipError_t e = hipSuccess;
  if (offsets) e = h->d2h(offsets, h->u_offsets(), (nc + 1) * 8);
  if (e == hipSuccess && seqs && nb) e = h->d2h(seqs, h->d_useq.p, nb);
  if (e == hipSuccess && depths && nc) e = h->d2h(depths, h->u_depths(), nc * 8);
  if (e == hipSuccess && n_kmers && nc) e = h->d2h(n_kmers, h->u_nkmers(), nc * 4);
  if (e == hipSuccess) e = hipStreamSynchronize(h->stream);
  return e == hipSuccess ? MHMKC_OK : h->hip_fail(e, "uutigs D2H");
}

int mhmkc_uutig_rows_device(mhmkc_t h, const uint32_t **d_row_ctg, const uint32_t **d_row_pos, const uint8_t **d_row_rc) {
  int rc = uutigs_need(h);
  if (rc) return rc;
  const uint64_t n = h->n_out;
  const size_t rows_b = align_up(n * 4, 256);
  const char *base = n ? h->d_urows.as<char>() : nullptr;
  if (d_row_ctg) *d_row_ctg = (const uint32_t *)base;
  if (d_row_pos) *d_row_pos = base ? (const uint32_t *)(base + rows_b) : nullptr;
  if (d_row_rc) *d_row_rc = base ? (const uint8_t *)(base + 2 * rows_b) : nullptr;
  return MHMKC_OK;
}

int mhmkc_uutig_rows(mhmkc_t h, uint32_t *row_ctg, uint32_t *row_pos, uint8_t *row_rc) {
  const uint32_t *dc = nullptr, *dp = nullptr;
  const uint8_t *dr = nullptr;
  int rc = mhmkc_uutig_rows_device(h, &dc, &dp, &dr);
  if (rc) return rc;
  const uint64_t n = h->n_out;
  if (!n) return MHMKC_OK;
  hipError_t e = hipSuccess;
  if (row_ctg) e = h->d2h(row_ctg, dc, n * 4);
  if (e == hipSuccess && row_pos) e = h->d2h(row_pos, dp, n * 4);
  if (e == hipSuccess && row_rc) e = h->d2h(row_rc, dr, n);
  if (e == hipSuccess) e = hipStreamSynchronize(h->stream);
  return e == hipSuccess ? MHMKC_OK : h->hip_fail(e, "uutig rows D2H");
}

int mhmkc_uutigs_info(mhmkc_t h, mhmkc_uutig_info *info) {
  if (!h || !info) return MHMKC_EINVAL;
  *info = h->uinfo;
  return MHMKC_OK;
}

int mhmkc_get_stats(mhmkc_t h, mhmkc_stats *s) {
  if (!h || !s) return MHMKC_EINVAL;
  *s = h->st;
  return MHMKC_OK;
}

int mhmkc_reset(mhmkc_t h) {
  if (!h) return MHMKC_EINVAL;
  hipError_t e = hipStreamSynchronize(h->stream);
  if (e == hipSuccess && h->xstream) e = hipStreamSynchronize(h->xstream);
  if (e == hipSuccess && h->pstream) e = hipStreamSynchronize(h->pstream);
  if (e != hipSuccess) return h->hip_fail(e, "reset");
  h->inc = h->inc_tried = false;
  h->inc_parted = 0;
  h->inc_expect = h->inc_announced = h->x_expect_all = h->x_r0_total = 0;
  h->x_r0_coarse.clear();
  h->x_round_slab.clear();
  h->lq = 0;
  h->inc_distinct = h->inc_ext_per_rec = 0;
  h->prof_collect();
  h->n_slabs = 0;
  h->n_parts = 0;
  h->xq = 0;
  h->x_rounds = 0;
  h->x_all_done = false;
  h->n_arenas = 0;
  h->ctg_bytes.clear();
  h->ctg_offs.assign(1, 0);
  h->ctg_win.assign(1, 0);
  h->ctg_depth.clear();
  h->ctg_n = 0;
  h->fq_reads = h->fq_bases = 0;
  h->finished = false;
  h->began = false;
  h->partial = false;
  h->n_out = 0;
  h->ord_ready = false;
  const bool had_query = h->d_qidx.p || h->d_links.p || h->d_qstage.p || h->d_uctg.p || h->d_urows.p || h->d_useq.p;
  h->drop_query();
  memset(&h->st, 0, sizeof h->st);
  if (had_query) {
    h->st.device_bytes = g_dev_live.load();
    h->st.device_bytes_peak = g_dev_peak.load();
  }
  if ((e = hipMemsetAsync(h->d_err.p, 0, 16, h->stream)) != hipSuccess) return h->hip_fail(e, "reset");
  return MHMKC_OK;
}

int mhmkc_set_profiling(mhmkc_t h, int on) {
  if (!h) return MHMKC_EINVAL;
  h->profiling = on != 0;
  h->prof_heavy_only = on == 2;
  return MHMKC_OK;
}

const char *mhmkc_last_error(mhmkc_t h) { return h ? h->err.c_str() : g_create_error.c_str(); }

int mhmkc_debug_set(const char *knob, int64_t value) {
  if (!knob) return MHMKC_EINVAL;
  const std::string k = knob;
  if (k == "exact") g_dbg.exact = value;
  else if (k == "cap") g_dbg.cap = value;
  else if (k == "fine_bits") g_dbg.fine_bits = value;
  else if (k == "out_cap") g_dbg.out_cap = value;
  else if (k == "fq_read_fail") g_dbg.fq_read_fail = value;
  else if (k == "wide_records") g_dbg.wide_records = value;
  else if (k == "smer") g_dbg.smer = value;
  else if (k == "chunk_bytes") g_dbg.chunk_bytes = value;
  else if (k == "d2h_chunk") g_dbg.d2h_chunk = value;
  else if (k == "h2d_nib") g_dbg.h2d_nib = value;
  else if (k == "local_rounds") g_dbg.local_rounds = value;
  else if (k == "h2d_threads") g_dbg.h2d_threads = value;
  else if (k == "h2d_nt") g_dbg.h2d_nt = value;
  else if (k == "h2d_adapt") g_dbg.h2d_adapt = value;
  else if (k == "cb0") g_dbg.cb0[1] = value;
  else if (k == "cb0_2") g_dbg.cb0[2] = value;
  else if (k == "cb0_3") g_dbg.cb0[3] = value;
  else if (k == "query_slots_log2") g_dbg.query_slots_log2 = value;
  else if (k == "query_grid") mhm::query_grid_cap = (unsigned)std::max<int64_t>(0, std::min<int64_t>(value, 16384));
  else if (k == "merge_grid") mhm::merge_grid_cap = (unsigned)std::max<int64_t>(0, std::min<int64_t>(value, 16384));
  else return MHMKC_EINVAL;
  return MHMKC_OK;
}

void mhmkc_debug_reset(void) {
  g_dbg = DebugKnobs();
  mhm::query_grid_cap = 0;
  mhm::merge_grid_cap = 0;
}

int mhmkc_debug_nib_pack(const uint8_t *src, uint64_t n, uint8_t *dst, int qcut, int mode) {
  if ((!src || !dst) && n) return MHMKC_EINVAL;
  if (mode == 0) {
    nib_pack(src, n, dst, qcut);
  } else if (mode == 1) {
    nib_pack_swar(src, n, dst, qcut);
  } else if (mode == 2) {
    if (!__builtin_cpu_supports("avx2")) return MHMKC_EUNSUPPORTED;
    nib_pack_avx2(src, n, dst, qcut, false);
  } else {
    return MHMKC_EINVAL;
  }
  return MHMKC_OK;
}

}
```

Baseline: 110.7 billion.

## Pack small device results into a pinned mailbox and launch the distinct sketch early

Stats, error flags, output cursor and window counts now live in one contiguous device block. Each is read or armed with a single pinned-memory copy instead of several small copies and memsets. A new early sketch kernel reads extracted records straight from the slab planes before slab resolution and overlaps with it, replacing a later sketch launch and its blocking synchronisation. The window count becomes a running total to avoid a per-add memset. This adds persistent pinned buffers and more complex eligibility logic.

```diff
diff --git a/mhm2_proxy_amd/csrc/kcount_kernels.hip b/mhm2_proxy_amd/csrc/kcount_kernels.hip
--- a/mhm2_proxy_amd/csrc/kcount_kernels.hip
+++ b/mhm2_proxy_amd/csrc/kcount_kernels.hip
@@ -1386,6 +1386,61 @@
     if (reg[i]) {
       atomicMax(&hll[i], reg[i]);
       if (!(blockIdx.x & 1u)) atomicMax(&hll[SKETCH_M + 1 + i], reg[i]);
+    }
+  if (threadIdx.x == 0 && s_ext) atomicAdd(&hll[SKETCH_M], s_ext);
+}
+
+template <int NL, bool PACKED, bool CMP>
+__global__ __launch_bounds__(kPThreads<NL>()) void k_sketch_early(EarlySketch p, unsigned int *hll) {
+  constexpr int NT = kPThreads<NL>(), T = kPTile<NL>(), W = T / NT;
+  __shared__ unsigned int reg[SKETCH_M];
+  __shared__ unsigned int s_ext;
+  const uint32_t S = p.n_src, NP = S * E_NSUB;
+  auto pair_count = [&](uint32_t jj) -> uint64_t {
+    const uint32_t q = jj / S, sl = jj % S;
+    const uint64_t cur = p.cursor[sl][(uint64_t)q * p.n_bins + p.coarse];
+    const uint64_t base = ((uint64_t)p.coarse * E_NSUB + q) * p.cap[sl];
+    const uint64_t n = cur > base ? cur - base : 0;
+    return n < p.cap[sl] ? n : p.cap[sl];
+  };
+  uint32_t j = 0;
+  while (j + 1 < NP && blockIdx.x >= p.slot0[j + 1]) j++;
+  const uint32_t i = blockIdx.x - p.slot0[j];
+  const uint64_t cnt = pair_count(j);
+  if ((uint64_t)i * T >= cnt) return;
+  uint32_t chunk = i;
+  for (uint32_t jj = 0; jj < j; jj++) chunk += (uint32_t)((pair_count(jj) + T - 1) / T);
+  if (threadIdx.x == 0) s_ext = 0;
+  for (int x = threadIdx.x; x < SKETCH_M; x += NT) reg[x] = 0;
+  SChunk ch;
+  ch.start = ((uint64_t)p.coarse * E_NSUB + j / S) * p.cap[j % S] + (uint64_t)i * T;
+  ch.count = (uint32_t)(cnt - (uint64_t)i * T < (uint64_t)T ? cnt - (uint64_t)i * T : (uint64_t)T);
+  ch.src = j % S;
+  ch.coarse_local = 0;
+  ch.pad = 0;
+  const PlaneSet src = p.planes[j % S];
+  uint64_t rk[W][NL];
+  uint32_t re[W];
+  load_chunk<NL, PACKED, CMP, W>(src, ch, rk, re);
+  __syncthreads();
+  const uint64_t low_mask = CMP ? 63ull : PACKED ? (1ull << (EXT_BITS + p.hbits)) - 1 : 0ull;
+  uint32_t ext_adds = 0;
+#pragma unroll
+  for (int w_ = 0; w_ < W; w_++) {
+    if (threadIdx.x + w_ * NT >= ch.count) continue;
+    ext_adds += (uint32_t)(((re[w_] >> 3) & 7u) < 4u) + (uint32_t)((re[w_] & 7u) < 4u);
+    uint64_t h = 0x9E3779B97F4A7C15ull;
+#pragma unroll
+    for (int w = 0; w < NL; w++) h = fmix64(h ^ (w == RecKind<NL, CMP>::XW ? rk[w_][w] & ~low_mask : rk[w_][w]));
+    const uint32_t rho = (uint32_t)__clzll(h | (uint64_t)(SKETCH_M - 1)) + 1;
+    atomicMax(&reg[h & (SKETCH_M - 1)], rho);
+  }
+  atomicAdd(&s_ext, ext_adds);
+  __syncthreads();
+  for (int x = threadIdx.x; x < SKETCH_M; x += NT)
+    if (reg[x]) {
+      atomicMax(&hll[x], reg[x]);
+      if (!(chunk & 1u)) atomicMax(&hll[SKETCH_M + 1 + x], reg[x]);
     }
   if (threadIdx.x == 0 && s_ext) atomicAdd(&hll[SKETCH_M], s_ext);
 }
@@ -2807,6 +2862,26 @@
   MHM_DISPATCH(nl, packed, do_sketch, (p, n_chunks, hll, fine_hist, s));
 }
 
+template <int NL, bool PK, bool CMP = false>
+static hipError_t do_sketch_early(const EarlySketch &p, uint32_t n, unsigned int *hll, hipStream_t s) {
+  k_sketch_early<NL, PK, CMP><<<dim3(n), dim3(kPThreads<NL>()), 0, s>>>(p, hll);
+  return hipGetLastError();
+}
+
+hipError_t launch_sketch_early(EarlySketch &p, unsigned int *hll, int nl, bool packed, bool mixed, hipStream_t s) {
+  if (!p.n_src || p.n_src > (uint32_t)ES_MAX) return hipErrorInvalidValue;
+  const uint64_t T = (uint64_t)chunk_records(nl);
+  uint64_t n = 0;
+  for (uint32_t j = 0; j < p.n_src * E_NSUB; j++) {
+    p.slot0[j] = (uint32_t)n;
+    n += (p.cap[j % p.n_src] + T - 1) / T;
+  }
+  p.slot0[p.n_src * E_NSUB] = (uint32_t)n;
+  if (!n || n >= 0x7fffffffull) return hipErrorInvalidValue;
+  if (mixed) return MHM_DISPATCH_MIXED(nl, do_sketch_early, (p, (uint32_t)n, hll, s));
+  MHM_DISPATCH(nl, packed, do_sketch_early, (p, (uint32_t)n, hll, s));
+}
+
 hipError_t launch_scan(const unsigned long long *in, unsigned long long *base, unsigned long long *cursor, uint32_t n,
                        hipStream_t s) {
   k_scan<<<dim3(1), dim3(1024), 0, s>>>(in, base, cursor, n);
diff --git a/mhm2_proxy_amd/csrc/kcount_launch.hpp b/mhm2_proxy_amd/csrc/kcount_launch.hpp
--- a/mhm2_proxy_amd/csrc/kcount_launch.hpp
+++ b/mhm2_proxy_amd/csrc/kcount_launch.hpp
@@ -243,6 +243,16 @@
 constexpr int SKETCH_FB = 11, SKETCH_FH = 1 << SKETCH_FB;
 hipError_t launch_sketch(const PartitionParams &p, uint32_t n_chunks, unsigned int *hll, int nl, bool packed,
                          hipStream_t s, bool fine_hist = false);
+constexpr int ES_MAX = 8;
+struct EarlySketch {
+  PlaneSet planes[ES_MAX];
+  const unsigned long long *cursor[ES_MAX];
+  uint64_t cap[ES_MAX];
+  uint32_t slot0[ES_MAX * E_NSUB + 1];
+  uint32_t n_src, n_bins, coarse;
+  int hbits;
+};
+hipError_t launch_sketch_early(EarlySketch &p, unsigned int *hll, int nl, bool packed, bool mixed, hipStream_t s);
 hipError_t launch_scan(const unsigned long long *in, unsigned long long *base, unsigned long long *cursor,
                        uint32_t n, hipStream_t s);
 hipError_t launch_count(const CountParams &p, int nl, bool packed, hipStream_t s);
diff --git a/mhm2_proxy_amd/csrc/mhmkc_host.cpp b/mhm2_proxy_amd/csrc/mhmkc_host.cpp
--- a/mhm2_proxy_amd/csrc/mhmkc_host.cpp
+++ b/mhm2_proxy_amd/csrc/mhmkc_host.cpp
@@ -50,6 +50,8 @@
   int64_t local_rounds = 1;
   int64_t h2d_nib = -1;
   int64_t cb0[4] = {0, 0, 0, 0};
+  int64_t step_mailbox = 1;
+  int64_t step_sketch = 1;
   int64_t query_slots_log2 = 0;
 };
 DebugKnobs g_dbg;
@@ -87,6 +89,14 @@
   }
 };
 
+struct DevView {
+  void *p = nullptr;
+  template <class T>
+  T *as() const {
+    return (T *)p;
+  }
+};
+
 struct PinBuf {
   void *p = nullptr;
   size_t cap = 0;
@@ -123,6 +133,7 @@
   mhm::PlaneSet planes{};
   mhm::ReadsView rv{};
   uint64_t wins = 0;
+  uint64_t cap_seg = 0;
   uint64_t n = 0;
   uint32_t tiles = 0;
   int qcut = 20;
@@ -396,8 +407,21 @@
   bool nib_used[3] = {false, false, false};
   hipEvent_t stage_ev[2] = {nullptr, nullptr};
   int add_host_nib(const uint8_t *bytes, const uint64_t *offs, uint64_t n_reads, int qcut, uint64_t chunk);
-  DevBuf d_hist, d_tiles, d_tsb, d_err, d_stats, d_fine_hist, d_fine_base, d_fine_cursor, d_chunks, d_srcs;
-  DevBuf d_r2, d_out_keys, d_out_counts, d_out_left, d_out_right, d_out_cursor, d_recv, d_xg;
+  DevBuf d_hist, d_tiles, d_tsb, d_fine_hist, d_fine_base, d_fine_cursor, d_chunks;
+  DevBuf d_r2, d_out_keys, d_out_counts, d_out_left, d_out_right, d_recv, d_xg;
+  static constexpr size_t RES_STATS = 8 * mhm::STAT_ALLOC, RES_FIN = RES_STATS + 16 + 16, RES_ADD = 16 + 16;
+  static constexpr size_t RES_ALL = RES_FIN + 16;
+  uint64_t wins_seen = 0;
+  DevBuf d_res;
+  DevView d_stats, d_out_cursor, d_err, d_wins;
+  PinBuf pin_add, pin_fin, pin_arm, pin_tab, pin_hll;
+  static constexpr size_t HLL_BYTES = (4 * (size_t)mhm::SKETCH_WORDS + 15) / 16 * 16;
+  hipEvent_t ev_sketch = nullptr;
+  bool sketch_early_ok() const;
+  int sketch_early();
+  hipError_t arm_count(unsigned long long cur0);
+  hipError_t read_count(unsigned long long *stats, unsigned int &errf, unsigned long long &cursor_end, uint8_t *skip,
+                        size_t n_skip);
   DevBuf d_hll, d_dest, d_ohist, d_out2_keys, d_out2_counts, d_out2_left, d_out2_right, d_mh;
   DevBuf d_ord;
   mhm::OutRows ord{};
@@ -698,11 +722,13 @@
     }
     sl->bases[nseg] = tot;
     p.bin_cap = 0;
+    sl->cap_seg = 0;
   } else {
     const uint64_t expect = sl->wins / nseg;
     const uint64_t cap = align_up(expect + expect / 25 + 1024, 64);
     for (uint32_t i = 0; i <= nseg; i++) sl->bases[i] = (uint64_t)std::min(std::max(i, blo * NSUB), bhi * NSUB) * cap;
     p.bin_cap = cap;
+    sl->cap_seg = cap;
     shift = (uint64_t)blo * NSUB * cap;
   }
   int rc;
@@ -729,17 +755,26 @@
 int mhmkc::add_view(const mhm::ReadsView &rv, uint64_t wins, bool wins_known) {
   hipError_t e;
   if (!wins_known) {
-    if ((e = grow(d_hist, (size_t)nb * 8 + 64)) != hipSuccess) return hip_fail(e, "histogram");
-    unsigned long long *d_wins = d_hist.as<unsigned long long>() + nb;
+    unsigned long long *dw = d_wins.as<unsigned long long>();
+    prof_begin(MHMKC_STAGE_TILEIDX);
+    e = mhm::launch_count_windows(rv, k, dw, d_err.as<unsigned int>(), stream);
+    prof_end();
     unsigned int ef = 0;
-    prof_begin(MHMKC_STAGE_TILEIDX);
-    e = hipMemsetAsync(d_wins, 0, 8, stream);
-    if (e == hipSuccess) e = mhm::launch_count_windows(rv, k, d_wins, d_err.as<unsigned int>(), stream);
-    prof_end();
-    if (e == hipSuccess) e = hipMemcpyAsync(&wins, d_wins, 8, hipMemcpyDeviceToHost, stream);
-    if (e == hipSuccess) e = hipMemcpyAsync(&ef, d_err.p, 4, hipMemcpyDeviceToHost, stream);
-    if (e == hipSuccess) e = hipStreamSynchronize(stream);
+    unsigned long long wsum = 0;
+    if (g_dbg.step_mailbox) {
+      char *m = pin_add.as<char>();
+      if (e == hipSuccess) e = hipMemcpyAsync(m, d_err.p, RES_ADD, hipMemcpyDeviceToHost, stream);
+      if (e == hipSuccess) e = hipStreamSynchronize(stream);
+      memcpy(&ef, m, 4);
+      memcpy(&wsum, m + 16, 8);
+    } else {
+      if (e == hipSuccess) e = hipMemcpyAsync(&wsum, dw, 8, hipMemcpyDeviceToHost, stream);
+      if (e == hipSuccess) e = hipMemcpyAsync(&ef, d_err.p, 4, hipMemcpyDeviceToHost, stream);
+      if (e == hipSuccess) e = hipStreamSynchronize(stream);
+    }
     if (e != hipSuccess) return hip_fail(e, "window count");
+    wins = wsum - wins_seen;
+    wins_seen = wsum;
     if (ef & 4u)
       return fail(MHMKC_EINVAL, "device read offsets are not a PackedReads CSR (offs[0] == 0, non-decreasing, reads "
                                 "<= 65535 bases, offs[n_reads] == n_bases)");
@@ -765,6 +800,39 @@
   if (smer) return smer_build(sl);
   int rc = extract(sl, g_dbg.exact != 0);
   return rc ? rc : pump();
+}
+
+hipError_t mhmkc::arm_count(unsigned long long cur0) {
+  if (!g_dbg.step_mailbox) {
+    hipError_t e = hipMemcpyAsync(d_out_cursor.p, &cur0, 8, hipMemcpyHostToDevice, stream);
+    return e != hipSuccess ? e : hipMemsetAsync(d_stats.p, 0, RES_STATS, stream);
+  }
+  memcpy(pin_arm.as<char>() + RES_STATS, &cur0, 8);
+  return hipMemcpyAsync(d_res.p, pin_arm.p, RES_STATS + 8, hipMemcpyHostToDevice, stream);
+}
+
+hipError_t mhmkc::read_count(unsigned long long *stats, unsigned int &errf, unsigned long long &cursor_end,
+                             uint8_t *skip, size_t n_skip) {
+  hipError_t e;
+  if (!g_dbg.step_mailbox) {
+    if ((e = hipMemcpyAsync(stats, d_stats.p, RES_STATS, hipMemcpyDeviceToHost, stream)) != hipSuccess ||
+        (e = hipMemcpyAsync(&errf, d_err.p, 4, hipMemcpyDeviceToHost, stream)) != hipSuccess ||
+        (e = hipMemcpyAsync(&cursor_end, d_out_cursor.p, 8, hipMemcpyDeviceToHost, stream)) != hipSuccess ||
+        (n_skip && (e = hipMemcpyAsync(skip, d_inc_skip.p, n_skip, hipMemcpyDeviceToHost, stream)) != hipSuccess))
+      return e;
+    return hipStreamSynchronize(stream);
+  }
+  if ((e = pin_fin.ensure(RES_FIN + n_skip)) != hipSuccess) return e;
+  char *m = pin_fin.as<char>();
+  if ((e = hipMemcpyAsync(m, d_res.p, RES_FIN, hipMemcpyDeviceToHost, stream)) != hipSuccess ||
+      (n_skip && (e = hipMemcpyAsync(m + RES_FIN, d_inc_skip.p, n_skip, hipMemcpyDeviceToHost, stream)) != hipSuccess) ||
+      (e = hipStreamSynchronize(stream)) != hipSuccess)
+    return e;
+  memcpy(stats, m, RES_STATS);
+  memcpy(&cursor_end, m + RES_STATS, 8);
+  memcpy(&errf, m + RES_STATS + 16, 4);
+  if (n_skip) memcpy(skip, m + RES_FIN, n_skip);
+  return hipSuccess;
 }
 
 int mhmkc::resolve_one(Slab *sl, bool &redo) {
@@ -2089,6 +2157,41 @@
   return MHMKC_OK;
 }
 
+bool mhmkc::sketch_early_ok() const {
+  if (!g_dbg.step_sketch || G() != 1 || smer || inc || (lrounds && lq > 0) || n_parts || g_dbg.exact) return false;
+  if (n_slabs < 1 || n_slabs > (size_t)mhm::ES_MAX) return false;
+  for (size_t s = 0; s < n_slabs; s++)
+    if (!slabs[s]->cap_seg || slabs[s]->recv || slabs[s]->bin_hi) return false;
+  return true;
+}
+
+int mhmkc::sketch_early() {
+  hipError_t e;
+  mhm::EarlySketch es{};
+  es.n_src = (uint32_t)n_slabs;
+  es.n_bins = nb;
+  es.coarse = own_lo;
+  es.hbits = hbits;
+  for (size_t s = 0; s < n_slabs; s++) {
+    es.planes[s] = slabs[s]->planes;
+    es.cursor[s] = slabs[s]->meta.as<unsigned long long>();
+    es.cap[s] = slabs[s]->cap_seg;
+  }
+  if (!ev_sketch && (e = hipEventCreateWithFlags(&ev_sketch, hipEventDisableTiming)) != hipSuccess)
+    return hip_fail(e, "sketch event");
+  if ((e = grow(d_hll, HLL_BYTES + 64)) != hipSuccess || (e = pin_hll.ensure(4 * mhm::SKETCH_M + 4)) != hipSuccess)
+    return hip_fail(e, "distinct sketch");
+  prof_begin(MHMKC_STAGE_OTHER);
+  if ((e = hipMemsetAsync(d_hll.p, 0, HLL_BYTES, stream)) != hipSuccess ||
+      (e = mhm::launch_sketch_early(es, d_hll.as<unsigned int>(), nl, packed, mixed(), stream)) != hipSuccess)
+    return hip_fail(e, "distinct sketch");
+  prof_end();
+  if ((e = hipMemcpyAsync(pin_hll.p, d_hll.p, 4 * mhm::SKETCH_M + 4, hipMemcpyDeviceToHost, stream)) != hipSuccess ||
+      (e = hipEventRecord(ev_sketch, stream)) != hipSuccess)
+    return hip_fail(e, "sketch D2H");
+  return MHMKC_OK;
+}
+
 int mhmkc::finish(uint64_t *n_out_ret) {
   if (partial) return fail(MHMKC_ESTATE, "a failed mhmkc_add_fastq_file left part of the file in this round; call mhmkc_reset");
   int rc = begin_round();
@@ -2096,7 +2199,10 @@
   ord_ready = false;
   drop_query();
   ctg_gathered = false;
+  bool early_sketch = sketch_early_ok();
+  if (early_sketch && (rc = sketch_early())) return rc;
   if ((rc = resolve_slabs())) return rc;
+  for (size_t s = 0; s < n_slabs && early_sketch; s++) early_sketch = slabs[s]->cap_seg != 0;
   hipError_t e;
   const uint32_t no = n_owned();
   std::vector<Source> srcs;
@@ -2218,8 +2324,7 @@
   auto grow_output = [&](uint64_t rows) -> int {
     hipError_t e_;
     if ((e_ = grow(d_out_keys, rows * 8 * nlo)) != hipSuccess || (e_ = grow(d_out_counts, rows * 2)) != hipSuccess ||
-        (e_ = grow(d_out_left, rows)) != hipSuccess || (e_ = grow(d_out_right, rows)) != hipSuccess ||
-        (e_ = grow(d_out_cursor, 8)) != hipSuccess)
+        (e_ = grow(d_out_left, rows)) != hipSuccess || (e_ = grow(d_out_right, rows)) != hipSuccess)
       return hip_fail(e_, "output");
     return MHMKC_OK;
   };
@@ -2258,8 +2363,7 @@
       unsigned long long stats[mhm::STAT_ALLOC], cursor_end = 0;
       const unsigned long long cur0 = 0;
       prof_begin(MHMKC_STAGE_OTHER);
-      e = hipMemcpyAsync(d_out_cursor.p, &cur0, 8, hipMemcpyHostToDevice, stream);
-      if (e == hipSuccess) e = hipMemsetAsync(d_stats.p, 0, 8 * mhm::STAT_ALLOC, stream);
+      e = arm_count(cur0);
       if (e == hipSuccess && ctg_n) e = hipMemsetAsync(d_ctg_done.p, 0, ctg_n, stream);
       prof_end();
       if (e != hipSuccess) return hip_fail(e, "count setup");
@@ -2268,12 +2372,7 @@
       prof_end();
       if (e != hipSuccess) return hip_fail(e, "count");
       (void)hipEventRecord(ev_end, stream);
-      if ((e = hipMemcpyAsync(stats, d_stats.p, sizeof stats, hipMemcpyDeviceToHost, stream)) != hipSuccess ||
-          (e = hipMemcpyAsync(&errf, d_err.p, 4, hipMemcpyDeviceToHost, stream)) != hipSuccess ||
-          (e = hipMemcpyAsync(&cursor_end, d_out_cursor.p, 8, hipMemcpyDeviceToHost, stream)) != hipSuccess ||
-          (e = hipMemcpyAsync(skip.data(), d_inc_skip.p, no, hipMemcpyDeviceToHost, stream)) != hipSuccess ||
-          (e = hipStreamSynchronize(stream)) != hipSuccess)
-        return hip_fail(e, "finish");
+      if ((e = read_count(stats, errf, cursor_end, skip.data(), no)) != hipSuccess) return hip_fail(e, "finish");
       if (errf & 32u) return fail(MHMKC_EUNSUPPORTED, CLAMP_LOG_FULL);
       if (errf & 2u) break;
       if (errf & 16u) {
@@ -2351,26 +2450,34 @@
     if (n_chunks >= 0x7fffffffull) return fail(MHMKC_EINVAL, "too many chunks");
     uint64_t xcd_max = 0;
     for (int x = 0; x < 8; x++) xcd_max = std::max(xcd_max, xcd_start[x + 1] - xcd_start[x]);
-    if ((e = grow(d_chunks, align_up(std::max<size_t>(1, runs.size()) * sizeof(mhm::SRun), 256) +
-                                sizeof(mhm::SChunk) * (n_chunks + 1) + 256)) !=
-        hipSuccess)
+    const size_t runs_b = align_up(std::max<size_t>(1, runs.size()) * sizeof(mhm::SRun), 256);
+    const size_t ps_b = align_up(std::max<size_t>(1, ps.size()) * sizeof(mhm::PlaneSet), 256);
+    if ((e = grow(d_chunks, runs_b + ps_b + sizeof(mhm::SChunk) * (n_chunks + 1) + 256)) != hipSuccess)
       return hip_fail(e, "chunk table");
     mhm::SRun *d_runs = d_chunks.as<mhm::SRun>();
-    mhm::SChunk *d_chunk_run = (mhm::SChunk *)(d_chunks.as<char>() + align_up(runs.size() * sizeof(mhm::SRun), 256));
-    if ((e = grow(d_srcs, std::max<size_t>(1, ps.size()) * sizeof(mhm::PlaneSet) + 64)) != hipSuccess ||
-        (e = grow(d_cfit, 16 * (size_t)np_ + 64)) != hipSuccess)
-      return hip_fail(e, "source table");
+    mhm::PlaneSet *d_ps = (mhm::PlaneSet *)(d_chunks.as<char>() + runs_b);
+    mhm::SChunk *d_chunk_run = (mhm::SChunk *)(d_chunks.as<char>() + runs_b + ps_b);
+    if ((e = grow(d_cfit, 16 * (size_t)np_ + 64)) != hipSuccess) return hip_fail(e, "layout table");
     unsigned long long *cfit_d = d_cfit.as<unsigned long long>();
-    if (!runs.empty()) {
-      if ((e = hipMemcpyAsync(d_runs, runs.data(), runs.size() * sizeof(mhm::SRun), hipMemcpyHostToDevice, stream)) !=
-          hipSuccess)
+    const bool mail = g_dbg.step_mailbox != 0;
+    if (mail && (e = pin_tab.ensure(runs_b + ps_b + 16 * (size_t)np_)) != hipSuccess) return hip_fail(e, "pinned tables");
+    if (mail) {
+      char *m = pin_tab.as<char>();
+      memset(m, 0, runs_b + ps_b);
+      if (!runs.empty()) memcpy(m, runs.data(), runs.size() * sizeof(mhm::SRun));
+      if (!ps.empty()) memcpy(m + runs_b, ps.data(), ps.size() * sizeof(mhm::PlaneSet));
+      if ((e = hipMemcpyAsync(d_runs, m, runs_b + ps_b, hipMemcpyHostToDevice, stream)) != hipSuccess)
         return hip_fail(e, "run table H2D");
-      if ((e = mhm::launch_chunk_runs(d_runs, (uint32_t)runs.size(), d_chunk_run, T, stream)) != hipSuccess)
-        return hip_fail(e, "chunk index");
-    }
-    if (!ps.empty() && (e = hipMemcpyAsync(d_srcs.p, ps.data(), ps.size() * sizeof(mhm::PlaneSet),
-                                           hipMemcpyHostToDevice, stream)) != hipSuccess)
-      return hip_fail(e, "source H2D");
+    } else {
+      if (!runs.empty() && (e = hipMemcpyAsync(d_runs, runs.data(), runs.size() * sizeof(mhm::SRun),
+                                               hipMemcpyHostToDevice, stream)) != hipSuccess)
+        return hip_fail(e, "run table H2D");
+      if (!ps.empty() && (e = hipMemcpyAsync(d_ps, ps.data(), ps.size() * sizeof(mhm::PlaneSet), hipMemcpyHostToDevice,
+                                             stream)) != hipSuccess)
+        return hip_fail(e, "source H2D");
+    }
+    if (!runs.empty() && (e = mhm::launch_chunk_runs(d_runs, (uint32_t)runs.size(), d_chunk_run, T, stream)) != hipSuccess)
+      return hip_fail(e, "chunk index");
 
     if (pass == 0 && !inc_done) {
       fb = 4;
@@ -2381,21 +2488,29 @@
         sp.chunks = d_chunk_run;
         sp.n_runs = (uint32_t)runs.size();
         sp.n_chunks = (uint32_t)n_chunks;
-        sp.srcs = d_srcs.as<mhm::PlaneSet>();
+        sp.srcs = d_ps;
         sp.k = k;
         sp.coarse_bits = cb;
         sp.hbits = hbits;
         sp.compact = mixed();
         std::vector<uint32_t> reg(mhm::SKETCH_M + 1);
-        prof_begin(MHMKC_STAGE_OTHER);
-        if ((e = grow(d_hll, 4 * mhm::SKETCH_WORDS + 64)) != hipSuccess ||
-            (e = hipMemsetAsync(d_hll.p, 0, 4 * mhm::SKETCH_WORDS, stream)) != hipSuccess ||
-            (e = mhm::launch_sketch(sp, (uint32_t)n_c0, d_hll.as<unsigned int>(), nl, packed, stream)) != hipSuccess)
-          return hip_fail(e, "distinct sketch");
-        prof_end();
-        if ((e = hipMemcpyAsync(reg.data(), d_hll.p, 4 * mhm::SKETCH_M + 4, hipMemcpyDeviceToHost, stream)) != hipSuccess ||
-            (e = hipStreamSynchronize(stream)) != hipSuccess)
-          return hip_fail(e, "sketch D2H");
+        if (mail && (e = pin_hll.ensure(4 * mhm::SKETCH_M + 4)) != hipSuccess) return hip_fail(e, "pinned sketch");
+        void *reg_dst = mail ? pin_hll.p : (void *)reg.data();
+        if (early_sketch) {
+          if ((e = hipEventSynchronize(ev_sketch)) != hipSuccess) return hip_fail(e, "sketch D2H");
+          memcpy(reg.data(), pin_hll.p, 4 * mhm::SKETCH_M + 4);
+        } else {
+          prof_begin(MHMKC_STAGE_OTHER);
+          if ((e = grow(d_hll, HLL_BYTES + 64)) != hipSuccess ||
+              (e = hipMemsetAsync(d_hll.p, 0, HLL_BYTES, stream)) != hipSuccess ||
+              (e = mhm::launch_sketch(sp, (uint32_t)n_c0, d_hll.as<unsigned int>(), nl, packed, stream)) != hipSuccess)
+            return hip_fail(e, "distinct sketch");
+          prof_end();
+          if ((e = hipMemcpyAsync(reg_dst, d_hll.p, 4 * mhm::SKETCH_M + 4, hipMemcpyDeviceToHost, stream)) != hipSuccess ||
+              (e = hipStreamSynchronize(stream)) != hipSuccess)
+            return hip_fail(e, "sketch D2H");
+          if (mail) memcpy(reg.data(), pin_hll.p, 4 * mhm::SKETCH_M + 4);
+        }
         if (per_coarse[0]) st.lds_ext_adds = (uint64_t)((double)reg[mhm::SKETCH_M] * (double)owned / (double)per_coarse[0]);
         reg.resize(mhm::SKETCH_M);
         est = hll_estimate(reg);
@@ -2420,7 +2535,8 @@
     const uint32_t n_fine = np_ * nf;
     st.fine_buckets += n_fine;
 
-    std::vector<uint64_t> cfit(2 * (size_t)np_);
+    std::vector<uint64_t> cfit_v(mail ? 0 : 2 * (size_t)np_);
+    uint64_t *cfit = mail ? (uint64_t *)(pin_tab.as<char>() + runs_b + ps_b) : cfit_v.data();
     uint64_t r2_size = 0;
     for (uint32_t c = 0; c < np_; c++) {
       const uint64_t ex = per_coarse[c] >> fb;
@@ -2429,7 +2545,7 @@
       cfit[np_ + c] = fcap;
       r2_size += fcap << fb;
     }
-    if ((e = hipMemcpyAsync(cfit_d, cfit.data(), 16 * (size_t)np_, hipMemcpyHostToDevice, stream)) != hipSuccess)
+    if ((e = hipMemcpyAsync(cfit_d, cfit, 16 * (size_t)np_, hipMemcpyHostToDevice, stream)) != hipSuccess)
       return hip_fail(e, "layout H2D");
     if ((e = grow(d_fine_hist, (size_t)n_fine * 8)) != hipSuccess) return hip_fail(e, "fine histogram");
     if ((e = grow(d_fine_base, (size_t)n_fine * 8)) != hipSuccess) return hip_fail(e, "fine bases");
@@ -2442,7 +2558,7 @@
     pp.n_chunks = (uint32_t)n_chunks;
     for (int x = 0; x < 9; x++) pp.xcd_start[x] = (uint32_t)xcd_start[x];
     pp.grid = (uint32_t)(8 * xcd_max);
-    pp.srcs = d_srcs.as<mhm::PlaneSet>();
+    pp.srcs = d_ps;
     pp.k = k;
     pp.coarse_bits = cb;
     pp.fine_bits = fb;
@@ -2471,8 +2587,7 @@
       cp.out_cap = out_cap;
       const unsigned long long cur0 = out_used;
       prof_begin(MHMKC_STAGE_OTHER);
-      e = hipMemcpyAsync(d_out_cursor.p, &cur0, 8, hipMemcpyHostToDevice, stream);
-      if (e == hipSuccess) e = hipMemsetAsync(d_stats.p, 0, 8 * mhm::STAT_ALLOC, stream);
+      e = arm_count(cur0);
       if (e == hipSuccess && ctg_n) e = hipMemsetAsync(d_ctg_done.p, 0, ctg_n, stream);
       if (e == hipSuccess && exact) e = hipMemsetAsync(d_fine_hist.p, 0, (size_t)n_fine * 8, stream);
       if (e == hipSuccess && !exact)
@@ -2507,11 +2622,7 @@
       prof_end();
       if (e != hipSuccess) return hip_fail(e, "count");
       (void)hipEventRecord(ev_end, stream);
-      if ((e = hipMemcpyAsync(stats, d_stats.p, sizeof stats, hipMemcpyDeviceToHost, stream)) != hipSuccess ||
-          (e = hipMemcpyAsync(&errf, d_err.p, 4, hipMemcpyDeviceToHost, stream)) != hipSuccess ||
-          (e = hipMemcpyAsync(&cursor_end, d_out_cursor.p, 8, hipMemcpyDeviceToHost, stream)) != hipSuccess ||
-          (e = hipStreamSynchronize(stream)) != hipSuccess)
-        return hip_fail(e, "finish");
+      if ((e = read_count(stats, errf, cursor_end, nullptr, 0)) != hipSuccess) return hip_fail(e, "finish");
       if (errf & 32u) return fail(MHMKC_EUNSUPPORTED, CLAMP_LOG_FULL);
       if (!(errf & (2u | 16u))) break;
       if (errf & 2u) {
@@ -2790,12 +2901,19 @@
   if ((e = hipStreamCreateWithFlags(&h->copy_stream, hipStreamNonBlocking)) != hipSuccess ||
       (e = hipEventCreate(&h->ev_begin)) != hipSuccess || (e = hipEventCreate(&h->ev_end)) != hipSuccess ||
       (e = hipEventCreate(&h->ev_h2d0)) != hipSuccess || (e = hipEventCreate(&h->ev_h2d1)) != hipSuccess ||
-      (e = h->d_err.ensure(16)) != hipSuccess || (e = h->d_stats.ensure(8 * mhm::STAT_ALLOC)) != hipSuccess ||
-      (e = hipMemset(h->d_err.p, 0, 16)) != hipSuccess) {
+      (e = h->d_res.ensure(mhmkc::RES_ALL)) != hipSuccess ||
+      (e = hipMemset(h->d_res.p, 0, mhmkc::RES_ALL)) != hipSuccess ||
+      (e = h->pin_add.ensure(mhmkc::RES_ADD)) != hipSuccess || (e = h->pin_fin.ensure(mhmkc::RES_FIN)) != hipSuccess ||
+      (e = h->pin_arm.ensure(mhmkc::RES_STATS + 8)) != hipSuccess) {
     g_create_error = std::string("init: ") + hipGetErrorString(e);
     mhmkc_destroy(h);
     return MHMKC_EHIP;
   }
+  h->d_stats.p = h->d_res.p;
+  h->d_out_cursor.p = h->d_res.as<char>() + mhmkc::RES_STATS;
+  h->d_err.p = h->d_res.as<char>() + mhmkc::RES_STATS + 16;
+  h->d_wins.p = h->d_res.as<char>() + mhmkc::RES_FIN;
+  memset(h->pin_arm.p, 0, mhmkc::RES_STATS + 8);
   const char *xp_env = getenv("MHMKC_XPIPE");
   h->xpipe = cfg->n_ranks > 1 && !h->smer && xp_env && atoi(xp_env);
   h->lrounds = cfg->n_ranks == 1 && !h->smer && g_dbg.local_rounds != 0;
@@ -2842,6 +2960,7 @@
   if (h->pstream) (void)hipStreamDestroy(h->pstream);
   if (h->ev_pdone) (void)hipEventDestroy(h->ev_pdone);
   if (h->ev_tail0) (void)hipEventDestroy(h->ev_tail0);
+  if (h->ev_sketch) (void)hipEventDestroy(h->ev_sketch);
   for (RecvPart *q : h->parts) {
     q->buf.release();
     delete q;
@@ -2863,9 +2982,9 @@
     a->offs.release();
     delete a;
   }
-  DevBuf *bufs[] = {&h->d_hist,     &h->d_tiles,      &h->d_err,        &h->d_stats,      &h->d_fine_hist,
-                    &h->d_fine_base, &h->d_fine_cursor, &h->d_chunks,    &h->d_srcs,       &h->d_r2,
-                    &h->d_out_keys, &h->d_out_counts, &h->d_out_left,   &h->d_out_right,  &h->d_out_cursor,
+  DevBuf *bufs[] = {&h->d_hist,     &h->d_tiles,      &h->d_res,        &h->d_fine_hist,
+                    &h->d_fine_base, &h->d_fine_cursor, &h->d_chunks,    &h->d_r2,
+                    &h->d_out_keys, &h->d_out_counts, &h->d_out_left,   &h->d_out_right,
                     &h->d_recv,     &h->d_xg,         &h->d_hll,        &h->d_dest,       &h->d_ohist,
                     &h->d_out2_keys, &h->d_out2_counts, &h->d_out2_left, &h->d_out2_right, &h->d_mh, &h->d_ord,
                     &h->d_spill,      &h->d_cfit,       &h->d_xsend,      &h->d_xsegs,
@@ -2883,6 +3002,7 @@
   h->x_send.release();
   h->x_recv.release();
   h->fq_file_buf.release();
+  for (PinBuf *b : {&h->pin_add, &h->pin_fin, &h->pin_arm, &h->pin_tab, &h->pin_hll}) b->release();
   for (auto &p : h->prof) {
     h->ev_pool.push_back(p.a);
     h->ev_pool.push_back(p.b);
@@ -4026,7 +4146,8 @@
     h->st.device_bytes = g_dev_live.load();
     h->st.device_bytes_peak = g_dev_peak.load();
   }
-  if ((e = hipMemsetAsync(h->d_err.p, 0, 16, h->stream)) != hipSuccess) return h->hip_fail(e, "reset");
+  h->wins_seen = 0;
+  if ((e = hipMemsetAsync(h->d_err.p, 0, mhmkc::RES_ADD, h->stream)) != hipSuccess) return h->hip_fail(e, "reset");
   return MHMKC_OK;
 }
 
@@ -4056,6 +4177,8 @@
   else if (k == "h2d_threads") g_dbg.h2d_threads = value;
   else if (k == "h2d_nt") g_dbg.h2d_nt = value;
   else if (k == "h2d_adapt") g_dbg.h2d_adapt = value;
+  else if (k == "step_mailbox") g_dbg.step_mailbox = value;
+  else if (k == "step_sketch") g_dbg.step_sketch = value;
   else if (k == "cb0") g_dbg.cb0[1] = value;
   else if (k == "cb0_2") g_dbg.cb0[2] = value;
   else if (k == "cb0_3") g_dbg.cb0[3] = value;
```

Result: no change. 111.6 billion, median of 6 (+0.8%).
